# Scalsol/mega.pytorch

Hardware: NVIDIA H100
Metric: frames/sec MEGA R-101 inference (1000x600) (higher is better)
Workload: dtype f16 hi + f16 lo split operands, 3 products (near-f32) / f32 accumulate

## Files before the change

include/mega_b200.h:

```cpp
#ifndef MEGA_B200_H_
#define MEGA_B200_H_

#include <stdint.h>

#ifdef __cplusplus
extern "C" {
#endif

const char* mega_last_error(void);
int mega_abi_version(void);
int mega_device_ok(void);

typedef struct mega_conv_gemm_desc {
  const void* a;
  int a_n, a_h, a_w, a_c;
  long long a_stride_w, a_stride_h, a_stride_n;
  const void* b;
  int b_n, b_k;
  long long b_stride_n, b_stride_tap;
  int taps_r, taps_s, dil, pad;
  int k_per_tap;
  void* out;
  long long out_ld;
  int n_img, out_h, out_w, cout;
  const float* scale;
  const float* bias;
  const void* residual;
  long long res_ld;
  int relu;
  int tile_h, tile_w, block_n;
  int batch;
  int a_c_off, a_n_off;
  int b_k_off, b_n_off;
  int out_c_off, out_n_off;
  int res_c_off, res_n_off;
  int bias_z_off;
  int precision;
  int max_ctas;
  int stream_k;
  void* workspace;
  long long workspace_bytes;
  int out_f16;
  int pdl;
  int stride_h, stride_w;
  int pad_w_set, pad_w;
  long long out_stride_h, out_stride_n;
  long long res_stride_h, res_stride_n;
  int b_lo_tap_off;
  int res_split;
  float acc_scale;
  int group_width;
} mega_conv_gemm_desc;

int mega_split16_pack(const float* src, void* dst, long long n_values, void* stream);
int mega_split16_unpack(const void* src, float* dst, long long n_values, void* stream);
int mega_conv_gemm(const mega_conv_gemm_desc* desc, void* stream);
int mega_conv_gemm_tf32(const mega_conv_gemm_desc* desc, void* stream);
long long mega_conv_gemm_workspace_bytes(void);

long long mega_conv_chain_plan_bytes(int n_layers);
int mega_conv_chain_encode(const mega_conv_gemm_desc* descs, int n_layers, void* plan_host, long long plan_bytes,
                           int* grid_out);
int mega_conv_chain_launch(const void* plan_device, int n_layers, int grid, void* sync_words, void* stream, int pdl);
int mega_conv_chain_encode2(const mega_conv_gemm_desc* descs, int n_layers, void* plan_host, long long plan_bytes,
                            int* grid_out, int depth);
int mega_conv_chain_launch2(const void* plan_device, int n_layers, int grid, void* sync_words, void* stream, int pdl,
                            int depth);
int mega_conv_chain_set_trace(void* trace_dev, int cta);
int mega_conv_chain_set_trace2(void* trace_dev, int cta, int level);
int mega_set_split3_seg_len(int k_blocks);
int mega_set_tf32_rounding(int enable);

long long mega_nms_workspace_bytes(int n);
int mega_nms(const float* boxes , const float* scores , int n, float thresh, void* workspace,
             long long workspace_bytes, long long* keep_out , int* count_out, void* stream);

int mega_nms_host(const void* boxes , const void* scores , int n, float thresh, int is_double,
                  long long* keep_out , int* count_out);
int mega_roi_align_forward_nchw_host(const void* input, int batch, int channels, int height, int width, const void* rois,
                                     int num_rois, float spatial_scale, int pooled_h, int pooled_w, int sampling_ratio,
                                     int is_double, void* output);

long long mega_rpn_select_workspace_bytes(int n_img, int h, int w, int num_anchors, int pre_nms);
int mega_rpn_select(const float* head, long long head_img_stride, int ld, int n_img, int h, int w, int num_anchors,
                    int stride, const float* base_anchors, float im_w, float im_h, int pre_nms, int post_nms,
                    float nms_thresh, float min_size, void* workspace, long long workspace_bytes, float* out_boxes,
                    float* out_scores, int* out_anchor, int* out_count, void* stream);

int mega_roi_align_forward_nchw(const float* input, int batch, int channels, int height, int width,
                                const float* rois, int num_rois, float spatial_scale, int pooled_h, int pooled_w,
                                int sampling_ratio, float* output, void* stream);
int mega_roi_align_forward_nhwc(const float* input, int channels, int height, int width, long long in_img_stride,
                                const float* rois, int roi_ld, int roi_box_off, const int* roi_batch, int num_rois,
                                float spatial_scale, int pooled_h, int pooled_w, int sampling_ratio, float* output,
                                long long out_roi_stride, void* stream);

int mega_roi_align_forward_nhwc_f16(const void* input, int channels, int height, int width, long long in_img_stride,
                                    const float* rois, int roi_ld, int roi_box_off, const int* roi_batch,
                                    int num_rois, float spatial_scale, int pooled_h, int pooled_w, int sampling_ratio,
                                    void* output, long long out_roi_stride, void* stream);
int mega_roi_align_forward_nhwc_split16(const void* input, int channels, int height, int width, long long in_img_stride,
                                        const float* rois, int roi_ld, int roi_box_off, const int* roi_batch,
                                        int num_rois, float spatial_scale, int pooled_h, int pooled_w, int sampling_ratio,
                                        void* output, long long out_roi_stride, void* stream);

int mega_stem_im2col(const float* input, int n_img, int height, int width, int kpad, float* out, void* stream);
int mega_maxpool3x3s2_nhwc(const float* input, int n_img, int height, int width, int channels, float* out,
                           void* stream);
int mega_stem_im2col_f16(const float* input, int n_img, int height, int width, int kpad, void* out, void* stream);
int mega_maxpool3x3s2_nhwc_f16(const void* input, int n_img, int height, int width, int channels, void* out,
                               void* stream);
int mega_stem_prep(const float* input, int n_img, int height, int width, int wp, void* out, int f16, void* stream);
int mega_gather_rows(const float* src, long long src_ld, const int* idx, int n_rows, int row_len, float* dst,
                     long long dst_ld, void* stream);
int mega_copy_rows(const float* src, long long src_ld, const int* src_idx, float* dst, long long dst_ld,
                   const int* dst_idx, int n_rows, int row_len, void* stream);
typedef struct mega_copy_job {
  const void* src;
  long long src_ld;
  const int* src_idx;
  void* dst;
  long long dst_ld;
  const int* dst_idx;
  int n_rows;
  int row_len;
} mega_copy_job;
int mega_copy_rows_batch(const mega_copy_job* jobs_host, int n_jobs, void* stream);
int mega_transpose_2d(const float* input, int n_img, int rows, int cols, float* out, void* stream);

int mega_relation_softmax(float* logits, int n_rows, int ldm, const float* boxes_q, const float* boxes_k,
                          const float* wg, const float* bg, const float* dim_mat, const int* m_valid_ptr, int m_host,
                          const int* n_valid_ptr, int n_valid_off, float scale, void* stream);

int mega_relation_softmax_f16(float* logits, void* probs_f16, int n_rows, int ldm, const float* boxes_q,
                              const float* boxes_k, const float* wg, const float* bg, const float* dim_mat,
                              const int* m_valid_ptr, int m_host, const int* n_valid_ptr, int n_valid_off, float scale,
                              void* stream);

int mega_relation_softmax_pe(float* logits, void* probs_f16, int n_rows, int ldm, const float* boxes_q,
                             const float* boxes_k, const float* wg_host, const float* bg_host,
                             const float* dim_mat_host, const int* m_valid_ptr, int m_host, const int* n_valid_ptr,
                             int n_valid_off, float scale, void* stream);
int mega_relation_softmax_split16(float* logits, void* probs, int n_rows, int ldm, const float* boxes_q,
                                  const float* boxes_k, const float* wg, const float* bg, const float* dim_mat,
                                  const int* m_valid_ptr, int m_host, const int* n_valid_ptr, int n_valid_off, float scale,
                                  void* stream);
int mega_relation_softmax_pe_split16(float* logits, void* probs, int n_rows, int ldm, const float* boxes_q,
                                     const float* boxes_k, const float* wg_host, const float* bg_host,
                                     const float* dim_mat_host, const int* m_valid_ptr, int m_host, const int* n_valid_ptr,
                                     int n_valid_off, float scale, void* stream);

long long mega_box_postprocess_workspace_bytes(int r_max, int num_classes);
int mega_box_postprocess(const float* logits, int ld_logits, const float* deltas, int ld_deltas,
                         const float* proposals, const int* count_ptr, int r_max, int num_classes, float im_w,
                         float im_h, float score_thresh, float nms_thresh, int max_det, float wx, float wy, float ww,
                         float wh, void* workspace, long long workspace_bytes, float* out_boxes, float* out_scores,
                         long long* out_labels, int out_cap, int* out_count, void* stream);

int mega_fgfa_pool_image(const float* image, int height, int width, void* out, int f16, void* stream);
int mega_fgfa_build_pairs(const void* ring, long long slot_stride, const int* slots, int n_frames, int key_pos, int hq,
                          int wq, void* pairs, int f16, void* stream);
int mega_avgpool2_nhwc(const void* input, int n_img, int height, int width, int channels, long long in_ld, void* out,
                       long long out_ld, int f16, void* stream);
int mega_fgfa_aggregate(const void* ring, long long slot_stride, int ld, int feat_channels, int embed_channels,
                        const int* slots, int n_frames, int key_pos, const float* flow, int flow_ld, int height, int width,
                        void* out, long long out_ld, float* weights_out, int f16, void* stream);

int mega_dff_warp_scale(const void* key_feats, int ld, int channels, const float* flow, int flow_ld, const void* scale,
                        long long scale_ld, int height, int width, void* out, long long out_ld, int f16, void* stream);

int mega_sigmoid_focalloss_forward(const float* logits, const int* targets, int num_samples, int num_classes,
                                   float gamma, float alpha, float* losses, void* stream);
int mega_sigmoid_focalloss_backward(const float* logits, const int* targets, const float* d_losses, int num_samples,
                                    int num_classes, float gamma, float alpha, float* d_logits, void* stream);

int mega_deform_im2col(const float* input, const float* offset, const float* mask, int batch, int channels, int height,
                       int width, int kh, int kw, int pad_h, int pad_w, int stride_h, int stride_w, int dil_h, int dil_w,
                       int deformable_group, int kpad, float* cols, void* stream);

int mega_deform_psroi_pooling_forward(const float* input, const float* rois, const float* trans, int num_rois,
                                      int channels, int height, int width, int no_trans, float spatial_scale,
                                      int output_dim, int group_size, int pooled_size, int part_size,
                                      int sample_per_part, float trans_std, int num_classes, float* out,
                                      float* top_count, void* stream);


int mega_roi_align_backward_nchw(const float* grad, const float* rois, int num_rois, float spatial_scale, int pooled_h,
                                 int pooled_w, int batch, int channels, int height, int width, int sampling_ratio,
                                 float* grad_input, void* stream);

int mega_roi_pool_forward(const float* input, const float* rois, int num_rois, float spatial_scale, int channels,
                          int height, int width, int pooled_h, int pooled_w, float* output, int* argmax, void* stream);
int mega_roi_pool_backward(const float* grad, const int* argmax, const float* rois, int num_rois, int channels,
                           int height, int width, int pooled_h, int pooled_w, float* grad_input, void* stream);

int mega_deform_im2col_kq(const float* input, const float* offset, const float* mask, int batch, int channels,
                          int height, int width, int kh, int kw, int pad_h, int pad_w, int stride_h, int stride_w,
                          int dil_h, int dil_w, int deformable_group, int ldp, float* cols, void* stream);
int mega_deform_col2im_fused(const float* gcols, const float* input, const float* offset, const float* mask, int batch,
                             int channels, int height, int width, int kh, int kw, int pad_h, int pad_w, int stride_h,
                             int stride_w, int dil_h, int dil_w, int deformable_group, int ldp, float* grad_input,
                             float* grad_offset, float* grad_mask, void* stream);
int mega_channel_sum_nchw(const float* x, int batch, int channels, int plane, float* out, void* stream);

int mega_deform_psroi_pooling_backward(const float* out_grad, const float* input, const float* rois, const float* trans,
                                       const float* top_count, int num_rois, int channels, int height, int width,
                                       int no_trans, float spatial_scale, int output_dim, int group_size,
                                       int pooled_size, int part_size, int sample_per_part, float trans_std,
                                       int num_classes, float* input_grad, float* trans_grad, void* stream);

int mega_image_transform_u8(const unsigned char* src, int src_h, int src_w, long long src_row_stride,
                            long long src_pix_stride, long long src_ch_stride, const int* bounds_h, const int* kk_h, int ksize_h, const int* bounds_v, const int* kk_v, int ksize_v, int out_h,
                            int out_w, const float* mean_host, const float* std_host, int to_bgr255, float* out,
                            void* stream);
int mega_image_transform_u8_ex(const unsigned char* src, int src_h, int src_w, long long src_row_stride,
                               long long src_pix_stride, long long src_ch_stride, const int* bounds_h, const int* kk_h,
                               int ksize_h, const int* bounds_v, const int* kk_v, int ksize_v, int out_h, int out_w,
                               const float* mean_host, const float* std_host, int to_bgr255, int hflip, float* out,
                               void* stream);

int mega_vid_match_host(const float* pred_boxes, int n_pred, const float* gt_boxes, const unsigned char* gt_ignore,
                        int n_gt, float iou_thresh, double empty_weight, signed char* match_out,
                        double* pred_ignore_out);

long long mega_seq_nms_workspace_bytes(int num_frames, int max_det, int num_classes);
int mega_seq_nms(const float* boxes, const float* scores, const int* labels, const int* counts, int num_frames,
                 int max_det, const int* video_offsets, int num_videos, int num_classes, float link_iou, float nms_iou,
                 int rescore, void* workspace, long long workspace_bytes, float* out_scores, unsigned char* keep,
                 void* stream);

long long mega_bbox_aug_workspace_bytes(int num_passes, int r_max, int num_classes);
int mega_bbox_aug_collect(const float* logits, int ld_logits, const float* deltas, int ld_deltas, const float* proposals,
                          const int* count_ptr, int r_max, int num_classes, int pass, int num_passes, int im_w,
                          int im_h, int hflip, double ratio_w, double ratio_h, float score_thresh, float wx, float wy,
                          float ww, float wh, void* workspace, long long workspace_bytes, void* stream);
int mega_bbox_aug_merge(int num_passes, int r_max, int num_classes, float nms_thresh, int max_det, void* workspace,
                        long long workspace_bytes, float* out_boxes, float* out_scores, long long* out_labels,
                        int out_cap, int* out_count, void* stream);

#ifdef __cplusplus
}
#endif
#endif
```

mega.pytorch_b200/csrc/common.cuh:

```cuda
#pragma once
#include <cuda.h>
#include <cuda_runtime.h>
#include <stdint.h>
#include <stdio.h>

#define MEGA_OK 0
#define MEGA_ERR_ARG 1
#define MEGA_ERR_CUDA 2
#define MEGA_ERR_UNSUPPORTED 3

#define MEGA_CUDA_CHECK(expr)                                                      \
  do {                                                                             \
    cudaError_t _e = (expr);                                                       \
    if (_e != cudaSuccess) {                                                       \
      mega_set_error("%s:%d: %s -> %s", __FILE__, __LINE__, #expr,                 \
                     cudaGetErrorString(_e));                                      \
      return MEGA_ERR_CUDA;                                                        \
    }                                                                              \
  } while (0)

#define MEGA_ARG_CHECK(cond, ...)                                                  \
  do {                                                                             \
    if (!(cond)) {                                                                 \
      mega_set_error(__VA_ARGS__);                                                 \
      return MEGA_ERR_ARG;                                                         \
    }                                                                              \
  } while (0)

void mega_set_error(const char* fmt, ...);

static inline int mega_ceil_div(int a, int b) { return (a + b - 1) / b; }

#ifdef __CUDACC__
namespace mega {

__device__ __forceinline__ uint32_t smem_u32(const void* p) {
  return static_cast<uint32_t>(__cvta_generic_to_shared(p));
}

__device__ __forceinline__ uint32_t lane_id() { return threadIdx.x & 31; }

__device__ __forceinline__ bool elect_one() {
  uint32_t pred = 0;
  asm volatile(
      "{\n"
      ".reg .b32 rx;\n"
      ".reg .pred px;\n"
      "elect.sync rx|px, 0xffffffff;\n"
      "selp.b32 %0, 1, 0, px;\n"
      "}\n"
      : "=r"(pred));
  return pred != 0;
}

__device__ __forceinline__ void mbar_init(uint64_t* bar, uint32_t count) {
  asm volatile("mbarrier.init.shared::cta.b64 [%0], %1;" ::"r"(smem_u32(bar)), "r"(count));
}
__device__ __forceinline__ void fence_barrier_init() {
  asm volatile("fence.mbarrier_init.release.cluster;" ::: "memory");
}
__device__ __forceinline__ void mbar_arrive_expect_tx(uint64_t* bar, uint32_t bytes) {
  asm volatile("mbarrier.arrive.expect_tx.shared::cta.b64 _, [%0], %1;" ::"r"(smem_u32(bar)),
               "r"(bytes)
               : "memory");
}
__device__ __forceinline__ void mbar_arrive(uint64_t* bar) {
  asm volatile("mbarrier.arrive.shared::cta.b64 _, [%0];" ::"r"(smem_u32(bar)) : "memory");
}
__device__ __forceinline__ bool mbar_try_wait(uint64_t* bar, uint32_t parity) {
  uint32_t ok;
  asm volatile(
      "{\n"
      ".reg .pred p;\n"
      "mbarrier.try_wait.parity.shared::cta.b64 p, [%1], %2;\n"
      "selp.u32 %0, 1, 0, p;\n"
      "}\n"
      : "=r"(ok)
      : "r"(smem_u32(bar)), "r"(parity)
      : "memory");
  return ok != 0;
}
__device__ __forceinline__ uint64_t globaltimer_ns() {
  uint64_t t;
  asm volatile("mov.u64 %0, %%globaltimer;" : "=l"(t));
  return t;
}
__device__ __forceinline__ void mbar_wait(uint64_t* bar, uint32_t parity) {
  if (mbar_try_wait(bar, parity)) return;
#ifndef MEGA_NO_WATCHDOG
  uint64_t t0 = globaltimer_ns();
  uint32_t spins = 0;
#endif
  while (!mbar_try_wait(bar, parity)) {
#ifndef MEGA_NO_WATCHDOG
    if ((++spins & 0x3ff) == 0 && globaltimer_ns() - t0 > 2000000000ull) __trap();
#endif
  }
}

__device__ __forceinline__ void prefetch_tmap(const CUtensorMap* tm) {
  asm volatile("prefetch.tensormap [%0];" ::"l"(tm) : "memory");
}
__device__ __forceinline__ void tma_load_2d(void* dst, const CUtensorMap* tm, uint64_t* bar, int c0,
                                            int c1) {
  asm volatile(
      "cp.async.bulk.tensor.2d.shared::cluster.global.tile.mbarrier::complete_tx::bytes"
      " [%0], [%1, {%3, %4}], [%2];" ::"r"(smem_u32(dst)),
      "l"(tm), "r"(smem_u32(bar)), "r"(c0), "r"(c1)
      : "memory");
}
__device__ __forceinline__ void tma_load_3d(void* dst, const CUtensorMap* tm, uint64_t* bar, int c0,
                                            int c1, int c2) {
  asm volatile(
      "cp.async.bulk.tensor.3d.shared::cluster.global.tile.mbarrier::complete_tx::bytes"
      " [%0], [%1, {%3, %4, %5}], [%2];" ::"r"(smem_u32(dst)),
      "l"(tm), "r"(smem_u32(bar)), "r"(c0), "r"(c1), "r"(c2)
      : "memory");
}
__device__ __forceinline__ void tma_load_4d(void* dst, const CUtensorMap* tm, uint64_t* bar, int c0,
                                            int c1, int c2, int c3) {
  asm volatile(
      "cp.async.bulk.tensor.4d.shared::cluster.global.tile.mbarrier::complete_tx::bytes"
      " [%0], [%1, {%3, %4, %5, %6}], [%2];" ::"r"(smem_u32(dst)),
      "l"(tm), "r"(smem_u32(bar)), "r"(c0), "r"(c1), "r"(c2), "r"(c3)
      : "memory");
}

__device__ __forceinline__ void tma_store_4d(const CUtensorMap* tm, const void* src, int c0, int c1, int c2, int c3) {
  asm volatile(
      "cp.async.bulk.tensor.4d.global.shared::cta.bulk_group [%0, {%2, %3, %4, %5}], [%1];" ::"l"(tm),
      "r"(smem_u32(src)), "r"(c0), "r"(c1), "r"(c2), "r"(c3)
      : "memory");
}
__device__ __forceinline__ void tma_store_commit() { asm volatile("cp.async.bulk.commit_group;" ::: "memory"); }
template <int N>
__device__ __forceinline__ void tma_store_wait_read() {
  asm volatile("cp.async.bulk.wait_group.read %0;" ::"n"(N) : "memory");
}
template <int N>
__device__ __forceinline__ void tma_store_wait() {
  asm volatile("cp.async.bulk.wait_group %0;" ::"n"(N) : "memory");
}
__device__ __forceinline__ void fence_async_smem() { asm volatile("fence.proxy.async.shared::cta;" ::: "memory"); }

__device__ __forceinline__ void wgmma_fence() { asm volatile("wgmma.fence.sync.aligned;" ::: "memory"); }
__device__ __forceinline__ void wgmma_commit() { asm volatile("wgmma.commit_group.sync.aligned;" ::: "memory"); }
template <int N>
__device__ __forceinline__ void wgmma_wait() {
  asm volatile("wgmma.wait_group.sync.aligned %0;" ::"n"(N) : "memory");
}
template <int N>
__device__ __forceinline__ void wgmma_wait_regs(float (&d)[N]) {
#pragma unroll
  for (int i = 0; i < N; ++i) asm volatile("" : "+f"(d[i])::"memory");
}

template <int N>
__device__ __forceinline__ void setmaxnreg_dec() { asm volatile("setmaxnreg.dec.sync.aligned.u32 %0;" ::"n"(N)); }
template <int N>
__device__ __forceinline__ void setmaxnreg_inc() { asm volatile("setmaxnreg.inc.sync.aligned.u32 %0;" ::"n"(N)); }
__device__ __forceinline__ int ctaid_x_here() {
  int r;
  asm volatile("mov.u32 %0, %%ctaid.x;" : "=r"(r));
  return r;
}

__device__ __forceinline__ uint64_t wgmma_desc_sw128(uint32_t saddr) {
  uint64_t d = 0;
  d |= static_cast<uint64_t>((saddr & 0x3FFFFu) >> 4);
  d |= static_cast<uint64_t>(1) << 16;
  d |= static_cast<uint64_t>(1024 >> 4) << 32;
  d |= static_cast<uint64_t>(1) << 62;
  return d;
}

__device__ __forceinline__ void griddep_wait() { asm volatile("griddepcontrol.wait;" ::: "memory"); }
__device__ __forceinline__ void griddep_launch_dependents() { asm volatile("griddepcontrol.launch_dependents;" ::: "memory"); }

__device__ __forceinline__ uint32_t f2_to_h2(float lo, float hi) {
  uint32_t r;
  asm("cvt.rn.f16x2.f32 %0, %1, %2;" : "=r"(r) : "f"(hi), "f"(lo));
  return r;
}
__device__ __forceinline__ uint32_t f2_to_h2_sat(float lo, float hi) {
  uint32_t r;
  asm("cvt.rn.satfinite.f16x2.f32 %0, %1, %2;" : "=r"(r) : "f"(hi), "f"(lo));
  return r;
}
__device__ __forceinline__ float2 h2_to_f2(uint32_t h) {
  float2 f;
  asm("{\n.reg .b16 l, h;\nmov.b32 {l, h}, %2;\ncvt.f32.f16 %0, l;\ncvt.f32.f16 %1, h;\n}" : "=f"(f.x), "=f"(f.y) : "r"(h));
  return f;
}

__device__ __forceinline__ float4 ldg_f4(const float* p) {
  return __ldg(reinterpret_cast<const float4*>(p));
}

}
#endif
```

mega.pytorch_b200/csrc/conv_gemm.cu:

```cuda
#include "conv_gemm_kernel.cuh"

namespace mega {

template MEGA_LAUNCH_MODE(kModeTf32);
template MEGA_LAUNCH_MODE(kModeSplit3);

typedef CUresult (*EncodeTiledFn)(CUtensorMap*, CUtensorMapDataType, cuuint32_t, void*, const cuuint64_t*,
                                  const cuuint64_t*, const cuuint32_t*, const cuuint32_t*,
                                  CUtensorMapInterleave, CUtensorMapSwizzle, CUtensorMapL2promotion,
                                  CUtensorMapFloatOOBfill);

static EncodeTiledFn get_encode_fn() {
  static EncodeTiledFn fn = nullptr;
  if (fn) return fn;
  void* p = nullptr;
  cudaDriverEntryPointQueryResult qres;
  if (cudaGetDriverEntryPoint("cuTensorMapEncodeTiled", &p, cudaEnableDefault, &qres) != cudaSuccess ||
      qres != cudaDriverEntryPointSuccess || p == nullptr) {
    return nullptr;
  }
  fn = reinterpret_cast<EncodeTiledFn>(p);
  return fn;
}

static int g_tf32_round = 1;

static int g_num_sms = 0;
static int g_seg_len = 4;
constexpr int kCounterSlots = 65536;
constexpr int kMinUnits = 4;

}

using namespace mega;

extern "C" long long mega_conv_gemm_workspace_bytes(void) {
  return static_cast<long long>(kCounterSlots) * sizeof(int) +
         static_cast<long long>(kMaxCtas) * 2 * kBM * 256 * sizeof(float);
}

extern "C" int mega_set_split3_seg_len(int k_blocks) {
  int old = g_seg_len;
  if (k_blocks >= 1 && k_blocks <= 64) g_seg_len = k_blocks;
  return old;
}

extern "C" int mega_set_tf32_rounding(int enable) {
  int old = g_tf32_round;
  g_tf32_round = enable ? 1 : 0;
  return old;
}

namespace mega {

int encode_conv_gemm_problem(const mega_conv_gemm_desc* d, CUtensorMap* tmA_p, CUtensorMap* tmB_p, CUtensorMap* tmOut_p,
                             CUtensorMap* tmRes_p, ConvGemmParams* p_out, int* ctas_out) {
  MEGA_ARG_CHECK(d != nullptr, "conv_gemm: null descriptor");
  MEGA_ARG_CHECK(d->precision >= 0 && d->precision <= 3,
                 "conv_gemm: precision must be 0 (tf32), 1 (3xtf32), 2 (fp16 operands) or 3 (3xfp16, split-fp16 operands)");
  const bool strict = d->precision == kModeSplit3;
  const bool f16 = d->precision == kModeF16;
  const bool pk = d->precision == kModeF16x3;
  const bool out16 = d->out_f16 != 0 && !pk;
  const int esz = f16 ? 2 : 4;
  const int osz = out16 ? 2 : 4;
  const int ealign = 16 / esz, oalign = 16 / osz;
  const int bk = mode_bk(d->precision);
  MEGA_ARG_CHECK(d->tile_h > 0 && d->tile_w > 0 && d->tile_h * d->tile_w == kBM,
                 "conv_gemm: tile_h*tile_w must be 128 (got %dx%d)", d->tile_h, d->tile_w);
  MEGA_ARG_CHECK(d->tile_w <= 256 && d->tile_h <= 256, "conv_gemm: tile too large for a TMA box");
  const int stride_h = d->stride_h > 0 ? d->stride_h : 1, stride_w = d->stride_w > 0 ? d->stride_w : 1;
  MEGA_ARG_CHECK((d->tile_w - 1) * stride_w + 1 <= 256 && (d->tile_h - 1) * stride_h + 1 <= 256,
                 "conv_gemm: strided tile %dx%d (stride %dx%d) exceeds the 256-element TMA box", d->tile_h, d->tile_w,
                 stride_h, stride_w);
  MEGA_ARG_CHECK(d->block_n == 32 || d->block_n == 64 || d->block_n == 96 || d->block_n == 128 ||
                     d->block_n == 160 || d->block_n == 192 || d->block_n == 256,
                 "conv_gemm: block_n must be one of 32/64/96/128/160/192/256");
  MEGA_ARG_CHECK(!out16 || (f16 && d->block_n % 64 == 0),
                 "conv_gemm: fp16 output needs fp16 operands and block_n %% 64 == 0 (got precision %d, block_n %d)",
                 d->precision, d->block_n);
  MEGA_ARG_CHECK((reinterpret_cast<uintptr_t>(d->a) & 15) == 0 && (reinterpret_cast<uintptr_t>(d->b) & 15) == 0,
                 "conv_gemm: operand base pointers must be 16-byte aligned");
  MEGA_ARG_CHECK((d->a_stride_w % ealign) == 0 && (d->a_stride_h % ealign) == 0 && (d->a_stride_n % ealign) == 0,
                 "conv_gemm: activation strides must be multiples of 16 bytes");
  MEGA_ARG_CHECK(d->out != nullptr && (reinterpret_cast<uintptr_t>(d->out) & 15) == 0 && (d->out_ld % oalign) == 0,
                 "conv_gemm: output must be 16-byte aligned with a row pitch multiple of 16 bytes");
  MEGA_ARG_CHECK(d->residual == nullptr ||
                     ((reinterpret_cast<uintptr_t>(d->residual) & 15) == 0 && (d->res_ld % oalign) == 0),
                 "conv_gemm: residual must be 16-byte aligned with a row pitch multiple of 16 bytes");
  MEGA_ARG_CHECK(d->out_c_off == 0 || d->cout == d->block_n,
                 "conv_gemm: channel-offset batching needs cout == block_n (got %d vs %d)", d->cout, d->block_n);
  MEGA_ARG_CHECK((d->b_stride_n % ealign) == 0 && (d->b_stride_tap % ealign) == 0,
                 "conv_gemm: weight strides must be multiples of 16 bytes");
  MEGA_ARG_CHECK(d->batch >= 1, "conv_gemm: batch must be >= 1");
  MEGA_ARG_CHECK(d->workspace != nullptr && d->workspace_bytes >= mega_conv_gemm_workspace_bytes(),
                 "conv_gemm: workspace missing or smaller than mega_conv_gemm_workspace_bytes()");
  MEGA_ARG_CHECK((reinterpret_cast<uintptr_t>(d->workspace) & 255) == 0, "conv_gemm: workspace must be 256-byte aligned");
  EncodeTiledFn enc = get_encode_fn();
  if (!enc) {
    mega_set_error("conv_gemm: cuTensorMapEncodeTiled unavailable (no CUDA driver?)");
    return MEGA_ERR_CUDA;
  }
  MEGA_ARG_CHECK(!(strict || pk) || d->block_n == 64 || d->block_n == 128, "conv_gemm: 3xtf32 / 3xfp16 support block_n 64 / 128");
  if (pk) {
    MEGA_ARG_CHECK((d->a_c & 31) == 0 && (d->b_k & 31) == 0 && (d->k_per_tap & 31) == 0 && (d->a_c_off & 31) == 0 &&
                       (d->b_k_off & 31) == 0,
                   "conv_gemm: split-fp16 operands need channel counts / offsets in multiples of 32 (a_c %d, b_k %d, k %d)",
                   d->a_c, d->b_k, d->k_per_tap);
    const int cout_r = (d->cout + 31) & ~31;
    MEGA_ARG_CHECK(d->out_f16 == 0 || ((d->out_c_off & 31) == 0 && (d->cout == cout_r || (d->batch == 1 && d->out_ld >= cout_r))),
                   "conv_gemm: split-fp16 output needs cout (%d) in multiples of 32 (or batch 1 and a row pitch >= the rounded cout)", d->cout);
    MEGA_ARG_CHECK(d->res_split == 0 || d->residual == nullptr ||
                       ((d->res_c_off & 31) == 0 && (d->cout == cout_r || (d->batch == 1 && d->res_ld >= cout_r))),
                   "conv_gemm: split-fp16 residual needs cout (%d) in multiples of 32", d->cout);
    MEGA_ARG_CHECK((d->a_stride_w & 31) == 0 && (d->b_stride_n & 31) == 0 && (reinterpret_cast<uintptr_t>(d->a) & 127) == 0 &&
                       (reinterpret_cast<uintptr_t>(d->b) & 127) == 0,
                   "conv_gemm: split-fp16 operands need 128-byte aligned rows");
    MEGA_ARG_CHECK(d->scale == nullptr,
                   "conv_gemm: precision 3 takes no per-channel scale: fold it into the weights before packing them "
                   "(mega_core.b200.ops.pack_weights_split16(w, scale))");
  } else {
    MEGA_ARG_CHECK(d->res_split == 0, "conv_gemm: res_split needs precision 3");
  }
  if (d->group_width != 0) {
    const int gw = d->group_width;
    MEGA_ARG_CHECK(gw == 8 || gw == 16 || gw == 32 || gw == 64, "conv_gemm: group_width must be 8, 16, 32 or 64 (got %d)", gw);
    MEGA_ARG_CHECK(d->block_n == 64 && d->cout == 64 && d->k_per_tap == 64 && d->b_k == 64 && d->a_c_off == 64 &&
                       d->b_n_off == 64 && d->out_c_off == 64 && d->b_k_off == 0 && (d->residual == nullptr || d->res_c_off == 64),
                   "conv_gemm: group_width needs the 64-channel batched layout (block_n = cout = k_per_tap = b_k = 64, "
                   "a_c_off = b_n_off = out_c_off = res_c_off = 64, b_k_off = 0; got block_n %d cout %d k %d b_k %d offsets "
                   "%d %d %d %d %d)", d->block_n, d->cout, d->k_per_tap, d->b_k, d->a_c_off, d->b_n_off, d->out_c_off,
                   d->res_c_off, d->b_k_off);
    MEGA_ARG_CHECK(d->b_lo_tap_off == 0, "conv_gemm: group_width does not take pre-split weights (b_lo_tap_off)");
  }
  const CUtensorMapDataType dt = f16 ? CU_TENSOR_MAP_DATA_TYPE_FLOAT16
                                     : (g_tf32_round && !strict && !pk) ? CU_TENSOR_MAP_DATA_TYPE_TFLOAT32
                                                                 : CU_TENSOR_MAP_DATA_TYPE_FLOAT32;
  const CUtensorMapDataType odt = out16 ? CU_TENSOR_MAP_DATA_TYPE_FLOAT16 : CU_TENSOR_MAP_DATA_TYPE_FLOAT32;

  CUtensorMap& tmA = *tmA_p;
  CUtensorMap& tmB = *tmB_p;
  {
    cuuint64_t gdim[4] = {static_cast<cuuint64_t>(d->a_c), static_cast<cuuint64_t>(d->a_w),
                          static_cast<cuuint64_t>(d->a_h), static_cast<cuuint64_t>(d->a_n)};
    cuuint64_t gstr[3] = {static_cast<cuuint64_t>(d->a_stride_w) * esz, static_cast<cuuint64_t>(d->a_stride_h) * esz,
                          static_cast<cuuint64_t>(d->a_stride_n) * esz};
    cuuint32_t box[4] = {static_cast<cuuint32_t>(bk), static_cast<cuuint32_t>((d->tile_w - 1) * stride_w + 1),
                         static_cast<cuuint32_t>((d->tile_h - 1) * stride_h + 1), 1};
    cuuint32_t estr[4] = {1, static_cast<cuuint32_t>(stride_w), static_cast<cuuint32_t>(stride_h), 1};
    CUresult r = enc(&tmA, dt, 4, const_cast<void*>(d->a), gdim, gstr, box, estr, CU_TENSOR_MAP_INTERLEAVE_NONE,
                     CU_TENSOR_MAP_SWIZZLE_128B, CU_TENSOR_MAP_L2_PROMOTION_L2_256B,
                     CU_TENSOR_MAP_FLOAT_OOB_FILL_NONE);
    if (r != CUDA_SUCCESS) {
      mega_set_error("conv_gemm: encode A tensor map failed (CUresult %d) dims %d %d %d %d strides %lld %lld %lld",
                     static_cast<int>(r), d->a_c, d->a_w, d->a_h, d->a_n, d->a_stride_w, d->a_stride_h,
                     d->a_stride_n);
      return MEGA_ERR_CUDA;
    }
  }
  {
    const int taps = d->taps_r * d->taps_s;
    MEGA_ARG_CHECK(d->b_lo_tap_off == 0 || (strict && d->b_lo_tap_off == taps && d->batch == 1),
                   "conv_gemm: b_lo_tap_off (%d) needs precision 1, batch 1 and must equal taps_r * taps_s (%d)",
                   d->b_lo_tap_off, taps);
    cuuint64_t gdim[3] = {static_cast<cuuint64_t>(d->b_k), static_cast<cuuint64_t>(d->b_n),
                          static_cast<cuuint64_t>(taps + d->b_lo_tap_off)};
    cuuint64_t gstr[2] = {static_cast<cuuint64_t>(d->b_stride_n) * esz,
                          static_cast<cuuint64_t>((taps > 1 || d->b_lo_tap_off) && d->b_stride_tap > 0
                                                      ? d->b_stride_tap : d->b_stride_n * d->b_n) * esz};
    cuuint32_t box[3] = {static_cast<cuuint32_t>(bk), static_cast<cuuint32_t>(pass_n(d->block_n)), 1};
    cuuint32_t estr[3] = {1, 1, 1};
    CUresult r = enc(&tmB, dt, 3, const_cast<void*>(d->b), gdim, gstr, box, estr, CU_TENSOR_MAP_INTERLEAVE_NONE,
                     CU_TENSOR_MAP_SWIZZLE_128B, CU_TENSOR_MAP_L2_PROMOTION_L2_256B,
                     CU_TENSOR_MAP_FLOAT_OOB_FILL_NONE);
    if (r != CUDA_SUCCESS) {
      mega_set_error("conv_gemm: encode B tensor map failed (CUresult %d) dims %d %d %d strides %lld %lld",
                     static_cast<int>(r), d->b_k, d->b_n, taps, d->b_stride_n, d->b_stride_tap);
      return MEGA_ERR_CUDA;
    }
  }

  CUtensorMap& tmOut = *tmOut_p;
  CUtensorMap& tmRes = *tmRes_p;
  int out_cext = 0, out_tail0 = 0;
  long long out_str_h = 0, out_str_n = 0;
  {
    const int box_w = d->tile_w < 32 ? d->tile_w : 32;
    const int box_h = 32 / box_w;
    const int cw = out16 ? 64 : 32;
    for (int which = 0; which < 2; ++which) {
      const void* base = which == 0 ? d->out : d->residual;
      CUtensorMap* tm = which == 0 ? &tmOut : &tmRes;
      if (base == nullptr) {
        *tm = tmOut;
        continue;
      }
      const long long ld = which == 0 ? d->out_ld : d->res_ld;
      const int c_off = which == 0 ? d->out_c_off : d->res_c_off;
      const int n_off = which == 0 ? d->out_n_off : d->res_n_off;
      const bool split_fmt = pk && (which == 0 ? d->out_f16 != 0 : d->res_split != 0);
      const int c_extent = (split_fmt ? ((d->cout + 31) & ~31) : d->cout) + (d->batch - 1) * c_off;
      const int c_tail0 = (c_extent * osz / 16) * 16 / osz;
      if (which == 0) {
        out_cext = c_extent;
        out_tail0 = c_tail0;
      }
      const int c_map = (which == 0 && c_tail0 > 0) ? c_tail0 : c_extent;
      cuuint64_t gdim[4] = {static_cast<cuuint64_t>(c_map), static_cast<cuuint64_t>(d->out_w),
                            static_cast<cuuint64_t>(d->out_h),
                            static_cast<cuuint64_t>(d->n_img + (d->batch - 1) * n_off)};
      const long long sh = which == 0 ? d->out_stride_h : d->res_stride_h;
      const long long sn = which == 0 ? d->out_stride_n : d->res_stride_n;
      const long long str_h = sh > 0 ? sh : ld * d->out_w;
      const long long str_n = sn > 0 ? sn : str_h * d->out_h;
      MEGA_ARG_CHECK((str_h % oalign) == 0 && (str_n % oalign) == 0, "conv_gemm: output strides must be multiples of 16 bytes");
      if (which == 0) {
        out_str_h = str_h;
        out_str_n = str_n;
      }
      cuuint64_t gstr[3] = {static_cast<cuuint64_t>(ld) * osz, static_cast<cuuint64_t>(str_h) * osz,
                            static_cast<cuuint64_t>(str_n) * osz};
      cuuint32_t box[4] = {static_cast<cuuint32_t>(cw), static_cast<cuuint32_t>(box_w), static_cast<cuuint32_t>(box_h), 1};
      cuuint32_t estr[4] = {1, 1, 1, 1};
      CUresult r = enc(tm, odt, 4, const_cast<void*>(base), gdim, gstr, box, estr,
                       CU_TENSOR_MAP_INTERLEAVE_NONE, CU_TENSOR_MAP_SWIZZLE_128B, CU_TENSOR_MAP_L2_PROMOTION_L2_256B,
                       CU_TENSOR_MAP_FLOAT_OOB_FILL_NONE);
      if (r != CUDA_SUCCESS) {
        mega_set_error("conv_gemm: encode %s tensor map failed (CUresult %d): C %d W %d H %d N %d ld %lld",
                       which == 0 ? "output" : "residual", static_cast<int>(r), static_cast<int>(gdim[0]), d->out_w,
                       d->out_h, static_cast<int>(gdim[3]), ld);
        return MEGA_ERR_CUDA;
      }
    }
  }

  ConvGemmParams& p = *p_out;
  p.tile_w = d->tile_w;
  p.tile_h = d->tile_h;
  p.tiles_w = mega_ceil_div(d->out_w, d->tile_w);
  p.tiles_h = mega_ceil_div(d->out_h, d->tile_h);
  p.out_h = d->out_h;
  p.out_w = d->out_w;
  p.n_img = d->n_img;
  p.taps_r = d->taps_r;
  p.taps_s = d->taps_s;
  p.dil = d->dil;
  p.pad = d->pad;
  p.pad_w = d->pad_w_set ? d->pad_w : d->pad;
  p.stride_h = stride_h;
  p.stride_w = stride_w;
  p.k_chunks = mega_ceil_div(d->k_per_tap, bk);
  p.cout = d->cout;
  p.scale = d->scale;
  p.bias = d->bias;
  p.has_residual = d->residual != nullptr;
  p.relu = d->relu;
  p.a_c_off = d->a_c_off;
  p.a_n_off = d->a_n_off;
  p.b_k_off = d->b_k_off;
  p.b_n_off = d->b_n_off;
  p.out_c_off = d->out_c_off;
  p.out_n_off = d->out_n_off;
  p.res_c_off = d->res_c_off;
  p.res_n_off = d->res_n_off;
  p.bias_z_off = d->bias_z_off;
  p.box_w = d->tile_w < 32 ? d->tile_w : 32;
  p.box_h = 32 / p.box_w;
  p.m_tiles = p.tiles_w * p.tiles_h * p.n_img;
  p.n_tiles = mega_ceil_div(d->cout, d->block_n);
  p.kb_per_tile = d->taps_r * d->taps_s * p.k_chunks;
  const long long tiles = static_cast<long long>(d->batch) * p.m_tiles * p.n_tiles;
  p.total_units = tiles * p.kb_per_tile;
  p.total_tiles = tiles;
  p.stream_k = d->stream_k ? 1 : 0;
  p.seg_len = g_seg_len;
  p.b_lo_tap_off = d->b_lo_tap_off;
  p.res_split = d->res_split ? 1 : 0;
  p.acc_scale = (pk && d->acc_scale != 0.f) ? d->acc_scale : 1.f;
  p.out_ptr = d->out;
  p.out_ld = d->out_ld;
  p.out_str_h = out_str_h;
  p.out_str_n = out_str_n;
  p.out_tail0 = out_tail0;
  p.out_cext = out_cext;
  MEGA_ARG_CHECK(tiles <= kCounterSlots, "conv_gemm: %lld output tiles exceed the %d counter slots", tiles, kCounterSlots);
  MEGA_ARG_CHECK(p.total_units > 0, "conv_gemm: empty problem");
  MEGA_ARG_CHECK(p.total_units * kMaxCtas < (1LL << 31), "conv_gemm: %lld work units exceed the 32-bit work-list range",
                 p.total_units);
  p.counters = static_cast<int*>(d->workspace);
  p.part_ws = reinterpret_cast<float*>(static_cast<char*>(d->workspace) + kCounterSlots * sizeof(int));
  if (g_num_sms == 0) {
    int dev = 0;
    MEGA_CUDA_CHECK(cudaGetDevice(&dev));
    MEGA_CUDA_CHECK(cudaDeviceGetAttribute(&g_num_sms, cudaDevAttrMultiProcessorCount, dev));
    if (g_num_sms > kMaxCtas) g_num_sms = kMaxCtas;
  }
  long long ctas = p.stream_k ? p.total_units / kMinUnits : tiles;
  if (ctas < 1) ctas = 1;
  if (ctas > g_num_sms) ctas = g_num_sms;
  if (d->max_ctas > 0 && ctas > d->max_ctas) ctas = d->max_ctas;
  if (p.stream_k && p.kb_per_tile >= 256 && tiles <= ctas) {
    const long long aligned = (ctas / tiles) * tiles;
    if (aligned * 100 >= ctas * 85) ctas = aligned;
  }
  *ctas_out = static_cast<int>(ctas);
  return MEGA_OK;
}

}

extern "C" int mega_conv_gemm(const mega_conv_gemm_desc* d, void* stream_v) {
  cudaStream_t stream = static_cast<cudaStream_t>(stream_v);
  CUtensorMap tmA, tmB, tmOut, tmRes;
  ConvGemmParams p;
  int ctas = 0;
  const int erc = encode_conv_gemm_problem(d, &tmA, &tmB, &tmOut, &tmRes, &p, &ctas);
  if (erc != MEGA_OK) return erc;
  const bool out16 = d->out_f16 != 0;
  dim3 grid(static_cast<unsigned>(ctas), 1, 1);
  const int pdl = d->pdl ? 1 : 0;
  const int gw = d->group_width == 64 ? 0 : d->group_width;
  switch (d->precision) {
    case kModeTf32: return launch_mode<kModeTf32>(d->block_n, out16, gw, tmA, tmB, tmOut, tmRes, p, grid, stream, pdl);
    case kModeSplit3: return launch_mode<kModeSplit3>(d->block_n, out16, gw, tmA, tmB, tmOut, tmRes, p, grid, stream, pdl);
    case kModeF16: return launch_mode<kModeF16>(d->block_n, out16, gw, tmA, tmB, tmOut, tmRes, p, grid, stream, pdl);
    default: return launch_mode<kModeF16x3>(d->block_n, out16, gw, tmA, tmB, tmOut, tmRes, p, grid, stream, pdl);
  }
}

extern "C" int mega_conv_gemm_tf32(const mega_conv_gemm_desc* d, void* stream) { return mega_conv_gemm(d, stream); }
```

mega.pytorch_b200/csrc/conv_gemm_kernel.cuh:

```cuda
#include "common.cuh"
#pragma once
#include "mega_b200.h"
#include "wgmma.cuh"

namespace mega {

constexpr int kBM = 128;
constexpr int kModeTf32 = 0;
constexpr int kModeSplit3 = 1;
constexpr int kModeF16 = 2;
constexpr int kModeF16x3 = 3;
__host__ __device__ constexpr int mode_bk(int mode) { return mode == kModeF16 ? 64 : 32; }
constexpr int kThreads = 192;
constexpr int kMaxCtas = 132;
constexpr int kRingSlots = 2;
constexpr int kRingSlotBytes = kBM * 128;
__host__ __device__ constexpr int mma_warp0(int mode) { return mode == kModeSplit3 ? 12 : 8; }
__host__ __device__ constexpr int conv_gemm_threads(int mode) { return (mma_warp0(mode) + 8) * 32; }
constexpr int kF16x3RegsProducer = 40, kF16x3RegsEpilogue = 104, kF16x3RegsMma = 184;
static_assert(128 * kF16x3RegsProducer + 128 * kF16x3RegsEpilogue + 256 * kF16x3RegsMma == 65536 &&
                  conv_gemm_threads(kModeF16x3) == 512,
              "3xFP16 register split");
__host__ __device__ constexpr int pass_n(int bn) { return bn <= 128 ? bn : (bn == 160 ? 96 : bn / 2); }
constexpr int conv_gemm_stages(int mode, int bn) {
  if (mode == kModeSplit3) return bn == 64 ? 4 : 2;
  if (mode == kModeF16x3) return bn == 64 ? 5 : 4;
  return bn == 32 ? 6 : bn == 64 ? 5 : bn <= 128 ? 4 : bn <= 192 ? 3 : 2;
}

struct ConvGemmParams {
  int tiles_w, tiles_h, tile_w, tile_h;
  int out_h, out_w, n_img;
  int taps_r, taps_s, dil, pad;
  int pad_w;
  int stride_h, stride_w;
  int k_chunks;
  int cout;
  const float* scale;
  const float* bias;
  int has_residual;
  int relu;
  int a_c_off, a_n_off, b_k_off, b_n_off;
  int out_c_off, out_n_off;
  int res_c_off, res_n_off;
  int bias_z_off;
  int box_w, box_h;
  int m_tiles, n_tiles;
  int kb_per_tile;
  long long total_units;
  long long total_tiles;
  int stream_k;
  float* part_ws;
  int* counters;
  int seg_len;
  int b_lo_tap_off;
  int res_split;
  float acc_scale;
  void* out_ptr;
  long long out_ld, out_str_h, out_str_n;
  int out_tail0, out_cext;
};

template <int BN, int STAGES, int MODE = kModeTf32>
struct SmemLayout {
  static constexpr bool SPLIT3 = MODE == kModeSplit3;
  static constexpr int kABytes = kBM * 128;
  static constexpr int kBBytes = pass_n(BN) * 128;
  static constexpr int kHalf = kABytes + kBBytes;
  static constexpr int kStageBytes = SPLIT3 ? kHalf + kBBytes : kHalf;
  static constexpr int kRingOffset = STAGES * kStageBytes;
  static constexpr int kEpiOffset = kRingOffset + kRingSlots * kRingSlotBytes;
  static constexpr int kEpiBytes = 4 * 4 * 4096;
  static constexpr int kBarOffset = kEpiOffset + kEpiBytes;
  static constexpr int kSbCols = BN <= 128 ? 128 : 256;
  static constexpr int kSbOffset = kBarOffset + 512;
  static constexpr int kTotal = kSbOffset + 8 * kSbCols + 1024;
};

struct TileCoord {
  int img, h0, w0, n0, batch;
};

__device__ __forceinline__ TileCoord decode_tile(const ConvGemmParams& p, int t, int bn) {
  TileCoord c;
  const int m_tile = t % p.m_tiles;
  const int rest = t / p.m_tiles;
  const int n_tile = rest % p.n_tiles;
  c.batch = rest / p.n_tiles;
  const int tw_i = m_tile % p.tiles_w;
  const int th_i = (m_tile / p.tiles_w) % p.tiles_h;
  c.img = m_tile / (p.tiles_w * p.tiles_h);
  c.h0 = th_i * p.tile_h;
  c.w0 = tw_i * p.tile_w;
  c.n0 = n_tile * bn;
  return c;
}

__device__ __forceinline__ int cta_first_unit(int total, int grid, int c) {
  return static_cast<int>((static_cast<unsigned>(total) * static_cast<unsigned>(c)) / static_cast<unsigned>(grid));
}

__device__ __forceinline__ int unit_owner(int total, int grid, int u) {
  int c = static_cast<int>((static_cast<unsigned>(u) * static_cast<unsigned>(grid)) / static_cast<unsigned>(total));
  if (c >= grid) c = grid - 1;
  while (c + 1 < grid && cta_first_unit(total, grid, c + 1) <= u) ++c;
  while (c > 0 && cta_first_unit(total, grid, c) > u) --c;
  return c;
}

struct WorkIter {
  int u, u_end, tile, tiles;
  int KB, grid;
  bool sk;
  __device__ __forceinline__ WorkIter(const ConvGemmParams& p, int cta, int grid_)
      : tile(cta), tiles(static_cast<int>(p.total_tiles)), KB(p.kb_per_tile), grid(grid_), sk(p.stream_k != 0) {
    u = cta_first_unit(static_cast<int>(p.total_units), grid_, cta);
    u_end = cta_first_unit(static_cast<int>(p.total_units), grid_, cta + 1);
  }
  __device__ __forceinline__ bool next(int& t, int& kb0, int& kb1) {
    if (sk) {
      if (u >= u_end) return false;
      t = u / KB;
      kb0 = u - t * KB;
      kb1 = min(KB, kb0 + (u_end - u));
      u += kb1 - kb0;
      return true;
    }
    if (tile >= tiles) return false;
    t = tile;
    kb0 = 0;
    kb1 = KB;
    tile += grid;
    return true;
  }
};

template <int THREADS>
__device__ __forceinline__ void epi_bar_sync() { asm volatile("bar.sync 1, %0;" ::"n"(THREADS) : "memory"); }

__device__ __forceinline__ float* sk_part_row(const ConvGemmParams& p, int c, int slot, int row, int bn) {
  return p.part_ws + ((static_cast<long long>(c) * 2 + slot) * kBM + row) * bn;
}

__device__ __forceinline__ float* sk_own_part_row(const ConvGemmParams& p, int cta, int tile_item, int row, int bn) {
  return sk_part_row(p, cta, tile_item == 0 ? 0 : 1, row, bn);
}

__device__ __forceinline__ void sk_publish(float* part, int col0, const uint32_t (&acc)[32]) {
  float* ws = part + col0;
#pragma unroll
  for (int j = 0; j < 32; j += 4)
    __stcg(reinterpret_cast<float4*>(ws + j), make_float4(__uint_as_float(acc[j]), __uint_as_float(acc[j + 1]),
                                                          __uint_as_float(acc[j + 2]), __uint_as_float(acc[j + 3])));
}

template <int THREADS>
__device__ __forceinline__ bool sk_elect_finisher(const ConvGemmParams& p, int U, int grid, int KB, int t, int epi_tid,
                                                  int* flag, int& c_first, int& c_last) {
  __threadfence();
  epi_bar_sync<THREADS>();
  c_first = unit_owner(U, grid, t * KB);
  c_last = unit_owner(U, grid, t * KB + KB - 1);
  if (epi_tid == 0) {
    const int parts = c_last - c_first + 1;
    const int old = atomicAdd(&p.counters[t], 1);
    const int last = (old == parts - 1);
    if (last) p.counters[t] = 0;
    *flag = last;
  }
  epi_bar_sync<THREADS>();
  const bool finisher = *flag != 0;
  if (finisher) __threadfence();
  return finisher;
}

__device__ __forceinline__ void sk_reduce(const ConvGemmParams& p, int U, int grid, int KB, int t, int c_first, int c_last,
                                          int row, int bn, int col0, float (&acc)[32]) {
#pragma unroll
  for (int j = 0; j < 32; ++j) acc[j] = 0.f;
  for (int oc = c_first; oc <= c_last; ++oc) {
    const int slot = (cta_first_unit(U, grid, oc) >= t * KB) ? 0 : 1;
    const float* ws = sk_part_row(p, oc, slot, row, bn) + col0;
#pragma unroll
    for (int j = 0; j < 32; j += 4) {
      const float4 v = __ldcg(reinterpret_cast<const float4*>(ws + j));
      acc[j] += v.x; acc[j + 1] += v.y; acc[j + 2] += v.z; acc[j + 3] += v.w;
    }
  }
}

struct StoreBox {
  int w, h, res_n;
};
__device__ __forceinline__ StoreBox store_box(const ConvGemmParams& p, const TileCoord& tc, int q) {
  const int r0 = q * 32;
  const int bh0 = r0 / p.tile_w, bw0 = r0 - bh0 * p.tile_w;
  return {tc.w0 + bw0, tc.h0 + bh0, tc.img + tc.batch * p.res_n_off};
}

template <bool HALF>
__device__ __forceinline__ void store_tail(const ConvGemmParams& p, const uint8_t* rowp, int gc0, int cw, const StoreBox& box,
                                          int out_n, int lane) {
  const int h = box.h + lane / p.box_w, w = box.w + lane % p.box_w;
  if (h >= p.out_h || w >= p.out_w) return;
  const int j0 = max(p.out_tail0 - gc0, 0), j1 = min(p.out_cext - gc0, cw);
  const uint32_t sw = static_cast<uint32_t>(lane & 7);
  const long long pix = static_cast<long long>(out_n) * p.out_str_n + static_cast<long long>(h) * p.out_str_h +
                        static_cast<long long>(w) * p.out_ld + gc0;
  for (int j = j0; j < j1; ++j) {
    if (HALF)
      static_cast<uint16_t*>(p.out_ptr)[pix + j] =
          *reinterpret_cast<const uint16_t*>(rowp + ((static_cast<uint32_t>(j >> 3) ^ sw) << 4) + (j & 7) * 2);
    else
      static_cast<float*>(p.out_ptr)[pix + j] =
          *reinterpret_cast<const float*>(rowp + ((static_cast<uint32_t>(j >> 2) ^ sw) << 4) + (j & 3) * 4);
  }
}

__device__ __forceinline__ void stage_scale_bias(float* sb, int bias_off, const ConvGemmParams& p, const TileCoord& tc, int i) {
  const int n = tc.n0 + i;
  const int zoff = tc.batch * p.bias_z_off;
  sb[i] = (p.scale && n < p.cout) ? __ldg(p.scale + zoff + n) : 1.f;
  sb[bias_off + i] = (p.bias && n < p.cout) ? __ldg(p.bias + zoff + n) : 0.f;
}

struct PipeState {
  int stage;
  uint32_t phase;
};

template <int STAGES, class F>
__device__ __forceinline__ void produce_pass(const CUtensorMap* tmA, const CUtensorMap* tmB, uint64_t* full_bar,
                                             uint64_t* empty_bar, PipeState& ps, uint8_t* stage0, int stage_bytes, int b_off,
                                             int b_lo_off, int bk, uint32_t tx_bytes, const ConvGemmParams& p,
                                             const TileCoord& tc, int n0, int kb0, int kb1, int lane, F&& on_stage) {
  const int k_chunks = p.k_chunks, taps_s = p.taps_s;
  int tap = kb0 / k_chunks;
  int kc = kb0 - tap * k_chunks;
  int r = tap / taps_s;
  int sx = tap - r * taps_s;
  const int a_c0 = tc.batch * p.a_c_off, a_n = tc.img + tc.batch * p.a_n_off;
  const int b_k0 = tc.batch * p.b_k_off, b_n = n0 + tc.batch * p.b_n_off;
  for (int kb = kb0; kb < kb1; ++kb) {
    mbar_wait(&empty_bar[ps.stage], ps.phase ^ 1);
    on_stage(kb);
    uint8_t* dst = stage0 + ps.stage * stage_bytes;
    if (lane == 0) {
      mbar_arrive_expect_tx(&full_bar[ps.stage], tx_bytes);
      tma_load_4d(dst, tmA, &full_bar[ps.stage], kc * bk + a_c0, tc.w0 * p.stride_w + sx * p.dil - p.pad_w,
                  tc.h0 * p.stride_h + r * p.dil - p.pad, a_n);
    } else {
      tma_load_3d(dst + b_off, tmB, &full_bar[ps.stage], kc * bk + b_k0, b_n, tap);
      if (b_lo_off != 0) tma_load_3d(dst + b_lo_off, tmB, &full_bar[ps.stage], kc * bk + b_k0, b_n, tap + p.b_lo_tap_off);
    }
    if (++kc == k_chunks) {
      kc = 0;
      ++tap;
      if (++sx == taps_s) {
        sx = 0;
        ++r;
      }
    }
    if (++ps.stage == STAGES) {
      ps.stage = 0;
      ps.phase ^= 1;
    }
  }
}

__device__ __forceinline__ void ring_take(const uint8_t* ring, uint64_t* full, uint64_t* empty, uint32_t slot, uint32_t use,
                                          int row, uint32_t (&r)[32]) {
  mbar_wait(&full[slot], use & 1u);
  const uint8_t* rowp = ring + slot * kRingSlotBytes + row * 128;
#pragma unroll
  for (int j = 0; j < 8; ++j) {
    const uint4 v = *reinterpret_cast<const uint4*>(rowp + ((j ^ (row & 7)) << 4));
    r[4 * j] = v.x; r[4 * j + 1] = v.y; r[4 * j + 2] = v.z; r[4 * j + 3] = v.w;
  }
  __syncwarp();
  if ((threadIdx.x & 31) == 0) mbar_arrive(&empty[slot]);
}
__device__ __forceinline__ void ring_take(const uint8_t* ring, uint64_t* full, uint64_t* empty, uint32_t seq, int row,
                                          uint32_t (&r)[32]) {
  ring_take(ring, full, empty, seq % kRingSlots, seq / kRingSlots, row, r);
}
__device__ __forceinline__ void ring_skip(const uint8_t* ring, uint64_t* full, uint64_t* empty, uint32_t slot, uint32_t use,
                                          int row) {
  uint32_t r[32];
  ring_take(ring, full, empty, slot, use, row, r);
}
__device__ __forceinline__ void ring_skip(const uint8_t* ring, uint64_t* full, uint64_t* empty, uint32_t seq, int row) {
  ring_skip(ring, full, empty, seq % kRingSlots, seq / kRingSlots, row);
}

template <int NR>
__device__ __forceinline__ void ring_put(uint8_t* ring, uint64_t* full, uint64_t* empty, uint32_t slot, uint32_t use, int wg,
                                         int wtid, const float (&d)[NR], const int c) {
  if (use > 0) mbar_wait(&empty[slot], (use - 1) & 1u);
  const int r0 = wg * 64 + (wtid >> 5) * 16 + ((wtid & 31) >> 2);
  const int t = wtid & 3;
  uint8_t* base = ring + slot * kRingSlotBytes;
#pragma unroll
  for (int i = 0; i < 4; ++i) {
    const int j = 2 * i + (t >> 1);
    const int off = (t & 1) * 8;
    *reinterpret_cast<float2*>(base + r0 * 128 + ((j ^ (r0 & 7)) << 4) + off) =
        make_float2(d[4 * (4 * c + i)], d[4 * (4 * c + i) + 1]);
    const int r1 = r0 + 8;
    *reinterpret_cast<float2*>(base + r1 * 128 + ((j ^ (r1 & 7)) << 4) + off) =
        make_float2(d[4 * (4 * c + i) + 2], d[4 * (4 * c + i) + 3]);
  }
  mbar_arrive(&full[slot]);
}

template <int BN, int MODE>
__device__ __forceinline__ void mma_kblock(float (&d)[BN / 2], uint32_t a_addr, uint32_t b_addr, uint32_t b_lo_addr,
                                           const int wtid, const bool first) {
  const uint64_t adesc = wgmma_desc_sw128(a_addr);
  const uint64_t bdesc = wgmma_desc_sw128(b_addr);
  if constexpr (MODE == kModeSplit3) {
    const int g = (wtid >> 5) * 16 + ((wtid & 31) >> 2), t = wtid & 3;
    const uint64_t blo = wgmma_desc_sw128(b_lo_addr);
    uint32_t ahi[4][4], alo[4][4];
#pragma unroll
    for (int k = 0; k < 4; ++k) {
#pragma unroll
      for (int e = 0; e < 4; ++e) {
        const int r = g + (e & 1) * 8, col = 8 * k + t + (e >> 1) * 4;
        float x;
        asm volatile("ld.shared.f32 %0, [%1];" : "=f"(x) : "r"(a_addr + r * 128 + ((((col >> 2) ^ (r & 7)) << 4) | ((col & 3) << 2))));
        const uint32_t h = __float_as_uint(x) & 0xffffe000u;
        ahi[k][e] = h;
        alo[k][e] = __float_as_uint(x - __uint_as_float(h));
      }
    }
    wgmma_fence();
#pragma unroll
    for (int k = 0; k < 4; ++k) {
      Wgmma<BN>::tf32_rs(d, ahi[k], bdesc + 2 * k, (first && k == 0) ? 0 : 1);
      Wgmma<BN>::tf32_rs(d, ahi[k], blo + 2 * k, 1);
      Wgmma<BN>::tf32_rs(d, alo[k], bdesc + 2 * k, 1);
    }
  } else if constexpr (MODE == kModeF16x3) {
    wgmma_fence();
#pragma unroll
    for (int k = 0; k < 2; ++k) {
      Wgmma<BN>::f16_ss(d, adesc + 2 * k, bdesc + 2 * k, (first && k == 0) ? 0 : 1);
      Wgmma<BN>::f16_ss(d, adesc + 2 * k, bdesc + 4 + 2 * k, 1);
      Wgmma<BN>::f16_ss(d, adesc + 4 + 2 * k, bdesc + 2 * k, 1);
    }
  } else {
    wgmma_fence();
#pragma unroll
    for (int k = 0; k < 4; ++k) {
      if (MODE == kModeF16) Wgmma<BN>::f16_ss(d, adesc + 2 * k, bdesc + 2 * k, (first && k == 0) ? 0 : 1);
      else Wgmma<BN>::tf32_ss(d, adesc + 2 * k, bdesc + 2 * k, (first && k == 0) ? 0 : 1);
    }
  }
  wgmma_commit();
}

template <int V>
struct IntC {
  static constexpr int value = V;
};
template <int K, int KN, class F>
__device__ __forceinline__ void static_for(F&& f) {
  if constexpr (K < KN) {
    f(IntC<K>());
    static_for<K + 1, KN>(f);
  }
}

template <int MODE, int GW, int KC>
__device__ __forceinline__ void mma_kblock_grouped(float (&d)[32], uint32_t a_addr, uint32_t b_addr, uint32_t b_lo_addr,
                                                   const int wtid) {
  constexpr int KS = (MODE == kModeF16 || MODE == kModeF16x3) ? 16 : 8;
  constexpr int N = GW > KS ? GW : KS;
  constexpr int NK = MODE == kModeF16x3 ? 2 : 4;
  const uint64_t adesc = wgmma_desc_sw128(a_addr);
  const uint64_t bdesc = wgmma_desc_sw128(b_addr);
  if constexpr (MODE == kModeSplit3) {
    const int g = (wtid >> 5) * 16 + ((wtid & 31) >> 2), t = wtid & 3;
    const uint64_t blo = wgmma_desc_sw128(b_lo_addr);
    uint32_t ahi[4][4], alo[4][4];
#pragma unroll
    for (int k = 0; k < 4; ++k) {
#pragma unroll
      for (int e = 0; e < 4; ++e) {
        const int r = g + (e & 1) * 8, col = 8 * k + t + (e >> 1) * 4;
        float x;
        asm volatile("ld.shared.f32 %0, [%1];" : "=f"(x) : "r"(a_addr + r * 128 + ((((col >> 2) ^ (r & 7)) << 4) | ((col & 3) << 2))));
        const uint32_t h = __float_as_uint(x) & 0xffffe000u;
        ahi[k][e] = h;
        alo[k][e] = __float_as_uint(x - __uint_as_float(h));
      }
    }
    wgmma_fence();
    static_for<0, NK>([&](auto kc) {
      constexpr int k = decltype(kc)::value;
      constexpr int col0 = (32 * KC + KS * k) / N * N;
      float(&dd)[N / 2] = *reinterpret_cast<float(*)[N / 2]>(&d[col0 / 2]);
      Wgmma<N>::tf32_rs(dd, ahi[k], bdesc + 2 * k + 8 * col0, 1);
      Wgmma<N>::tf32_rs(dd, ahi[k], blo + 2 * k + 8 * col0, 1);
      Wgmma<N>::tf32_rs(dd, alo[k], bdesc + 2 * k + 8 * col0, 1);
    });
  } else {
    wgmma_fence();
    static_for<0, NK>([&](auto kc) {
      constexpr int k = decltype(kc)::value;
      constexpr int col0 = (32 * KC + KS * k) / N * N;
      float(&dd)[N / 2] = *reinterpret_cast<float(*)[N / 2]>(&d[col0 / 2]);
      if constexpr (MODE == kModeF16x3) {
        Wgmma<N>::f16_ss(dd, adesc + 2 * k, bdesc + 2 * k + 8 * col0, 1);
        Wgmma<N>::f16_ss(dd, adesc + 2 * k, bdesc + 4 + 2 * k + 8 * col0, 1);
        Wgmma<N>::f16_ss(dd, adesc + 4 + 2 * k, bdesc + 2 * k + 8 * col0, 1);
      } else if constexpr (MODE == kModeF16) {
        Wgmma<N>::f16_ss(dd, adesc + 2 * k, bdesc + 2 * k + 8 * col0, 1);
      } else {
        Wgmma<N>::tf32_ss(dd, adesc + 2 * k, bdesc + 2 * k + 8 * col0, 1);
      }
    });
  }
  wgmma_commit();
}

template <int MODE, int GW>
__device__ __forceinline__ void mma_kblock_grouped(float (&d)[32], uint32_t a_addr, uint32_t b_addr, uint32_t b_lo_addr,
                                                   const int wtid, const int kb) {
  if (mode_bk(MODE) == 64 || (kb & 1) == 0) mma_kblock_grouped<MODE, GW, 0>(d, a_addr, b_addr, b_lo_addr, wtid);
  else mma_kblock_grouped<MODE, GW, 1>(d, a_addr, b_addr, b_lo_addr, wtid);
}

struct MmaState {
  int stage;
  uint32_t phase;
  uint32_t uses[kRingSlots];
};

template <int PN, int STAGES, int MODE, class L, int GW = 0>
__device__ __forceinline__ void mma_pass(uint8_t* smem, uint64_t* full_bar, uint64_t* empty_bar, uint64_t* split_bar,
                                         uint8_t* ring, uint64_t* ring_full, uint64_t* ring_empty, MmaState& ms, int kb0,
                                         int kb1, int seg_len, int wg, int wtid, int hpc) {
  static_assert(GW == 0 || PN == 64, "grouped k-blocks need a 64-column pass");
  constexpr bool SPLIT3 = MODE == kModeSplit3;
  constexpr bool SEG = SPLIT3 || MODE == kModeF16x3;
  const int lane = wtid & 31;
  float d[PN / 2];
  float master[SEG ? PN / 2 : 1];
  if constexpr (MODE == kModeF16x3) {
#pragma unroll
    for (int i = 0; i < PN / 2; ++i) master[i] = -0.f;
  }
  bool has_master = false;
  for (int s0 = kb0, s1 = 0; s0 < kb1; s0 = s1) {
    s1 = (kb1 - s0 > seg_len) ? s0 + seg_len : kb1;
    int pending = -1;
    if constexpr (GW > 0) {
#pragma unroll
      for (int i = 0; i < PN / 2; ++i) d[i] = 0.f;
    }
    for (int kb = s0; kb < s1; ++kb) {
      mbar_wait(SPLIT3 ? &split_bar[ms.stage] : &full_bar[ms.stage], ms.phase);
      const uint32_t a_addr = smem_u32(smem + ms.stage * L::kStageBytes);
      if constexpr (GW > 0)
        mma_kblock_grouped<MODE, GW>(d, a_addr + wg * 64 * 128, a_addr + L::kABytes, a_addr + L::kABytes + L::kBBytes, wtid,
                                     kb);
      else
        mma_kblock<PN, MODE>(d, a_addr + wg * 64 * 128, a_addr + L::kABytes, a_addr + L::kABytes + L::kBBytes, wtid, kb == s0);
      if (SPLIT3) wgmma_wait<0>(); else wgmma_wait<1>();
      if (pending >= 0) {
        __syncwarp();
        if (lane == 0) mbar_arrive(&empty_bar[pending]);
      }
      pending = ms.stage;
      if (++ms.stage == STAGES) {
        ms.stage = 0;
        ms.phase ^= 1;
      }
    }
    wgmma_wait<0>();
    wgmma_wait_regs(d);
    if (pending >= 0) {
      __syncwarp();
      if (lane == 0) mbar_arrive(&empty_bar[pending]);
    }
    if constexpr (MODE == kModeF16x3) {
#pragma unroll
      for (int i = 0; i < PN / 2; ++i) master[i] = __fadd_rn(d[i], master[i]);
    } else if constexpr (SEG) {
#pragma unroll
      for (int i = 0; i < PN / 2; ++i) master[i] = has_master ? __fadd_rn(d[i], master[i]) : d[i];
      has_master = true;
    }
  }
#pragma unroll
  for (int c = 0; c < PN / 32; ++c) {
    uint32_t slot;
    if (hpc == 0) slot = (ms.uses[0] == ms.uses[1]) ? 0u : 1u;
    else slot = static_cast<uint32_t>((c / hpc) & 1);
    const uint32_t use = ms.uses[slot]++;
    if constexpr (SEG) ring_put(ring, ring_full, ring_empty, slot, use, wg, wtid, master, c);
    else ring_put(ring, ring_full, ring_empty, slot, use, wg, wtid, d, c);
  }
}

template <int BN, int STAGES, int MODE, bool OUT16, int GW = 0>
__global__ void __launch_bounds__(conv_gemm_threads(MODE), 1)
conv_gemm_kernel(const __grid_constant__ CUtensorMap tmA, const __grid_constant__ CUtensorMap tmB,
                      const __grid_constant__ CUtensorMap tmOut, const __grid_constant__ CUtensorMap tmRes,
                      const ConvGemmParams p) {
  constexpr bool SPLIT3 = MODE == kModeSplit3;
  constexpr bool PK = MODE == kModeF16x3;
  constexpr bool SEG = SPLIT3 || PK;
  constexpr bool OUTH = OUT16 && !PK;
  constexpr int kBK = mode_bk(MODE);
  constexpr int CW = OUTH ? 64 : 32;
  constexpr int kMmaWarp0 = mma_warp0(MODE);
  static_assert(!OUTH || BN % 64 == 0, "fp16 output needs block_n % 64 == 0");
  static_assert(SmemLayout<BN, STAGES, MODE>::kTotal <= 227 * 1024, "pipeline + staging exceed the 227 KB of a CTA");
  using L = SmemLayout<BN, STAGES, MODE>;
  const int kSegLen = SEG ? p.seg_len : 0x7fffffff;
  extern __shared__ uint8_t smem_raw[];
  uint8_t* smem = reinterpret_cast<uint8_t*>((reinterpret_cast<uintptr_t>(smem_raw) + 1023) &
                                             ~static_cast<uintptr_t>(1023));
  uint64_t* full_bar = reinterpret_cast<uint64_t*>(smem + L::kBarOffset);
  uint64_t* empty_bar = full_bar + STAGES;
  uint64_t* split_bar = empty_bar + STAGES;
  uint64_t* ring_full = split_bar + STAGES;
  uint64_t* ring_empty = ring_full + kRingSlots;
  uint64_t* res_bar = ring_empty + kRingSlots;
  int* epi_flag = reinterpret_cast<int*>(res_bar + 16);
  uint8_t* ring = smem + L::kRingOffset;

  const int warp = threadIdx.x >> 5;
  const int lane = threadIdx.x & 31;
  const int grid = gridDim.x;
  const int cta = blockIdx.x;
  const int U = static_cast<int>(p.total_units);
  const int KB = p.kb_per_tile;

  if (warp == 0 && lane == 0) {
    prefetch_tmap(&tmA);
    prefetch_tmap(&tmB);
    prefetch_tmap(&tmOut);
    if (p.has_residual) prefetch_tmap(&tmRes);
  }
  if (warp == 1 && lane == 0) {
    for (int s = 0; s < STAGES; ++s) {
      mbar_init(&full_bar[s], 1);
      mbar_init(&empty_bar[s], 8);
      mbar_init(&split_bar[s], 4);
    }
    for (int b = 0; b < kRingSlots; ++b) {
      mbar_init(&ring_full[b], 256);
      mbar_init(&ring_empty[b], 4);
    }
    for (int b = 0; b < 16; ++b) mbar_init(&res_bar[b], 1);
    fence_barrier_init();
  }
  __syncthreads();
  griddep_wait();
  griddep_launch_dependents();
  if (warp == 0) {
    if (PK) setmaxnreg_dec<kF16x3RegsProducer>();
    if (lane < 2) {
      PipeState ps = {0, 0};
      WorkIter it(p, PK ? ctaid_x_here() : cta, grid);
      int t;
      int kb0, kb1;
      const bool b_lo = SPLIT3 && p.b_lo_tap_off > 0;
      while (it.next(t, kb0, kb1)) {
        const TileCoord tc = decode_tile(p, t, BN);
        for (int pass = 0; pass < (BN > pass_n(BN) ? 2 : 1); ++pass)
          produce_pass<STAGES>(&tmA, &tmB, full_bar, empty_bar, ps, smem, L::kStageBytes, L::kABytes,
                               b_lo ? L::kABytes + L::kBBytes : 0, kBK, L::kHalf + (b_lo ? L::kBBytes : 0), p, tc,
                               tc.n0 + pass * pass_n(BN), kb0, kb1, lane, [](int) {});
      }
    }
  } else if (warp >= kMmaWarp0) {
    if (PK) setmaxnreg_inc<kF16x3RegsMma>();
    const int wg = (warp - kMmaWarp0) >> 2;
    const int wtid = threadIdx.x - (kMmaWarp0 + 4 * wg) * 32;
    constexpr int P0 = pass_n(BN), P1 = BN - P0;
    MmaState ms = {0, 0, {0, 0}};
    WorkIter it(p, PK ? ctaid_x_here() : cta, grid);
    int t;
    int kb0, kb1;
    while (it.next(t, kb0, kb1)) {
      mma_pass<P0, STAGES, MODE, L, GW>(smem, full_bar, empty_bar, split_bar, ring, ring_full, ring_empty, ms, kb0, kb1,
                                        kSegLen, wg, wtid, 0);
      if constexpr (P1 > 0)
        mma_pass<P1, STAGES, MODE, L>(smem, full_bar, empty_bar, split_bar, ring, ring_full, ring_empty, ms, kb0, kb1,
                                      kSegLen, wg, wtid, 0);
    }
  } else if (warp >= 6 && warp < 10 && !PK) {
    if (SPLIT3) {
      const int stid = threadIdx.x - kThreads;
      int stage = 0;
      uint32_t phase = 0;
      WorkIter it(p, cta, grid);
      int t;
      int kb0, kb1;
      const bool need_lo = p.b_lo_tap_off == 0;
      while (it.next(t, kb0, kb1)) {
        for (int kb = kb0; kb < kb1; ++kb) {
          mbar_wait(&full_bar[stage], phase);
          uint8_t* bb = smem + stage * L::kStageBytes + L::kABytes;
          constexpr int kVecs = L::kBBytes / 16;
#pragma unroll 4
          for (int v = stid; v < kVecs; v += 128) {
            float4 x = *reinterpret_cast<const float4*>(bb + v * 16);
            float4 h;
            h.x = __uint_as_float(__float_as_uint(x.x) & 0xffffe000u);
            h.y = __uint_as_float(__float_as_uint(x.y) & 0xffffe000u);
            h.z = __uint_as_float(__float_as_uint(x.z) & 0xffffe000u);
            h.w = __uint_as_float(__float_as_uint(x.w) & 0xffffe000u);
            *reinterpret_cast<float4*>(bb + v * 16) = h;
            if (need_lo)
              *reinterpret_cast<float4*>(bb + L::kBBytes + v * 16) = make_float4(x.x - h.x, x.y - h.y, x.z - h.z, x.w - h.w);
          }
          fence_async_smem();
          __syncwarp();
          if (lane == 0) mbar_arrive(&split_bar[stage]);
          if (++stage == STAGES) {
            stage = 0;
            phase ^= 1;
          }
        }
      }
    }
  } else if (PK && warp >= 4 && warp < 8) {
    setmaxnreg_dec<kF16x3RegsEpilogue>();
    constexpr int kCPW = BN / 32;
    const int q = warp & 3;
    const int row = q * 32 + lane;
    const int epi_tid = (warp - 4) * 32 + lane;
    uint8_t* stage_buf = smem + L::kEpiOffset + (warp - 4) * (kCPW * 4096);
    uint64_t* rbar = res_bar + (warp - 4) * 4;
    float* bias_s = reinterpret_cast<float*>(smem + L::kSbOffset);
    uint32_t rphase = 0;
    const int cta_e = ctaid_x_here();
    WorkIter it(p, cta_e, grid);
    int t;
    int kb0, kb1;
    uint32_t seq0 = 0;
    const uint32_t sw = static_cast<uint32_t>(lane & 7);
    const bool res_split = p.res_split != 0;
    const float slope = p.relu == 2 ? 0.1f : 0.f;
    for (int tile_item = 0; it.next(t, kb0, kb1); ++tile_item, seq0 += BN / 32) {
      const TileCoord tc = decode_tile(p, t, BN);
      const bool complete = (kb0 == 0 && kb1 == KB);
      const StoreBox box = store_box(p, tc, q);
      const int nchunks = min(BN / 32, (p.cout - tc.n0 + 31) / 32);
      const int bsel = tile_item & 1;
      epi_bar_sync<128>();
      if (tile_item == 0) {
        if (epi_tid < BN) {
          const int n = tc.n0 + epi_tid;
          bias_s[epi_tid] = (p.bias && n < p.cout) ? __ldg(p.bias + tc.batch * p.bias_z_off + n) : 0.f;
        }
        epi_bar_sync<128>();
      }
      float next_bias = 0.f;
      bool has_next = false;
      {
        WorkIter peek = it;
        int t2, k0, k1;
        has_next = peek.next(t2, k0, k1);
        if (has_next && epi_tid < BN) {
          const TileCoord tc2 = decode_tile(p, t2, BN);
          const int n = tc2.n0 + epi_tid;
          next_bias = (p.bias && n < p.cout) ? __ldg(p.bias + tc2.batch * p.bias_z_off + n) : 0.f;
        }
      }
      if (lane == 0) tma_store_wait_read<0>();
      __syncwarp();
      auto issue_residual = [&]() {
        if (p.has_residual && lane == 0) {
#pragma unroll
          for (int j = 0; j < kCPW; ++j) {
            if (j < nchunks) {
              mbar_arrive_expect_tx(&rbar[j], 4096);
              tma_load_4d(stage_buf + j * 4096, &tmRes, &rbar[j], tc.n0 + j * 32 + tc.batch * p.res_c_off, box.w, box.h,
                          box.res_n);
            }
          }
        }
      };
      if (complete) issue_residual();
      auto load_chunk = [&](const int j, float (&acc)[32]) {
        uint32_t raw[32];
        ring_take(ring, ring_full, ring_empty, seq0 + j, row, raw);
#pragma unroll
        for (int i = 0; i < 32; ++i) acc[i] = __uint_as_float(raw[i]);
      };
      bool finalize = complete;
      int c_first = cta_e, c_last = cta_e;
      if (!complete) {
        float* part = sk_own_part_row(p, cta_e, tile_item, row, BN);
#pragma unroll
        for (int j = 0; j < kCPW; ++j) {
          uint32_t raw[32];
          ring_take(ring, ring_full, ring_empty, seq0 + j, row, raw);
          sk_publish(part, j * 32, raw);
        }
        finalize = sk_elect_finisher<128>(p, U, grid, KB, t, epi_tid, epi_flag, c_first, c_last);
        if (finalize) issue_residual();
      }
      if (finalize) {
        const int out_n = tc.img + tc.batch * p.out_n_off;
#pragma unroll
        for (int j = 0; j < kCPW; ++j) {
          if (j < nchunks) {
            float acc[32];
            if (complete) load_chunk(j, acc);
            else sk_reduce(p, U, grid, KB, t, c_first, c_last, row, BN, j * 32, acc);
            uint8_t* rowp = stage_buf + j * 4096 + lane * 128;
            const float4* biv = reinterpret_cast<const float4*>(bias_s + bsel * BN + j * 32);
#pragma unroll
            for (int i = 0; i < 32; i += 4) {
              const float4 bi = biv[i >> 2];
              acc[i] = fmaf(acc[i], p.acc_scale, bi.x); acc[i + 1] = fmaf(acc[i + 1], p.acc_scale, bi.y);
              acc[i + 2] = fmaf(acc[i + 2], p.acc_scale, bi.z); acc[i + 3] = fmaf(acc[i + 3], p.acc_scale, bi.w);
            }
            if (p.has_residual) {
              mbar_wait(&rbar[j], (rphase >> j) & 1u);
              rphase ^= (1u << j);
              if (res_split) {
#pragma unroll
                for (int c = 0; c < 4; ++c) {
                  const uint4 rh = *reinterpret_cast<const uint4*>(rowp + ((static_cast<uint32_t>(c) ^ sw) << 4));
                  const uint4 rl = *reinterpret_cast<const uint4*>(rowp + ((static_cast<uint32_t>(4 + c) ^ sw) << 4));
                  const uint32_t hs[4] = {rh.x, rh.y, rh.z, rh.w}, ls[4] = {rl.x, rl.y, rl.z, rl.w};
#pragma unroll
                  for (int e = 0; e < 4; ++e) {
                    const float2 a2 = h2_to_f2(hs[e]), b2 = h2_to_f2(ls[e]);
                    acc[8 * c + 2 * e] += a2.x + b2.x;
                    acc[8 * c + 2 * e + 1] += a2.y + b2.y;
                  }
                }
              } else {
#pragma unroll
                for (int c = 0; c < 8; ++c) {
                  const float4 rr = *reinterpret_cast<const float4*>(rowp + ((static_cast<uint32_t>(c) ^ sw) << 4));
                  acc[4 * c] += rr.x; acc[4 * c + 1] += rr.y; acc[4 * c + 2] += rr.z; acc[4 * c + 3] += rr.w;
                }
              }
            }
            if (p.relu) {
#pragma unroll
              for (int i = 0; i < 32; ++i) acc[i] = fmaxf(acc[i], slope * acc[i]);
            }
            if (OUT16) {
#pragma unroll
              for (int c = 0; c < 4; ++c) {
                uint32_t hh[4], ll[4];
#pragma unroll
                for (int e = 0; e < 4; ++e) {
                  hh[e] = f2_to_h2_sat(acc[8 * c + 2 * e], acc[8 * c + 2 * e + 1]);
                  const float2 back = h2_to_f2(hh[e]);
                  ll[e] = f2_to_h2_sat(acc[8 * c + 2 * e] - back.x, acc[8 * c + 2 * e + 1] - back.y);
                }
                *reinterpret_cast<uint4*>(rowp + ((static_cast<uint32_t>(c) ^ sw) << 4)) = make_uint4(hh[0], hh[1], hh[2], hh[3]);
                *reinterpret_cast<uint4*>(rowp + ((static_cast<uint32_t>(4 + c) ^ sw) << 4)) = make_uint4(ll[0], ll[1], ll[2], ll[3]);
              }
            } else {
#pragma unroll
              for (int c = 0; c < 8; ++c)
                *reinterpret_cast<float4*>(rowp + ((static_cast<uint32_t>(c) ^ sw) << 4)) =
                    make_float4(acc[4 * c], acc[4 * c + 1], acc[4 * c + 2], acc[4 * c + 3]);
            }
            fence_async_smem();
            __syncwarp();
            const int gc0 = tc.n0 + j * 32 + tc.batch * p.out_c_off;
            if (!OUT16 && gc0 + 32 > p.out_tail0) store_tail<false>(p, rowp, gc0, 32, box, out_n, lane);
            if (lane == 0 && gc0 < p.out_tail0) {
              tma_store_4d(&tmOut, stage_buf + j * 4096, gc0, box.w, box.h, out_n);
              tma_store_commit();
            }
          } else if (complete) {
            ring_skip(ring, ring_full, ring_empty, seq0 + j, row);
          }
        }
      }
      if (has_next && epi_tid < BN) bias_s[(bsel ^ 1) * BN + epi_tid] = next_bias;
    }
    if (lane == 0) tma_store_wait<0>();
  } else if (PK) {
    setmaxnreg_dec<kF16x3RegsProducer>();
  } else if (warp >= 2 && warp < 6) {
    const int q = warp & 3;
    const int row = q * 32 + lane;
    const int epi_tid = (warp - 2) * 32 + lane;
    uint8_t* epi_out = smem + L::kEpiOffset + (warp - 2) * 16384;
    uint8_t* epi_res = epi_out + 8192;
    uint64_t* rbar = res_bar + (warp - 2) * 2;
    float* sb_s = reinterpret_cast<float*>(smem + L::kSbOffset);
    uint32_t rphase = 0;
    WorkIter it(p, cta, grid);
    int t;
    int kb0, kb1;
    uint32_t seq0 = 0;
    for (int tile_item = 0; it.next(t, kb0, kb1); ++tile_item, seq0 += BN / 32) {
      const TileCoord tc = decode_tile(p, t, BN);
      const bool complete = (kb0 == 0 && kb1 == KB);
      const StoreBox box = store_box(p, tc, q);
      const int nchunks = min(BN / CW, (p.cout - tc.n0 + CW - 1) / CW);
      epi_bar_sync<128>();
      for (int i = epi_tid; i < BN; i += 128) stage_scale_bias(sb_s, L::kSbCols, p, tc, i);
      if (complete && p.has_residual && lane == 0 && nchunks > 0) {
        mbar_arrive_expect_tx(&rbar[0], 4096);
        tma_load_4d(epi_res, &tmRes, &rbar[0], tc.n0 + tc.batch * p.res_c_off, box.w, box.h, box.res_n);
      }
      epi_bar_sync<128>();
      bool finalize = complete;
      int c_first = cta, c_last = cta;
      if (!complete) {
        float* part = sk_own_part_row(p, cta, tile_item, row, BN);
#pragma unroll 1
        for (int c = 0; c < BN / 32; ++c) {
          uint32_t raw[32];
          ring_take(ring, ring_full, ring_empty, seq0 + c, row, raw);
          sk_publish(part, c * 32, raw);
        }
        finalize = sk_elect_finisher<128>(p, U, grid, KB, t, epi_tid, epi_flag, c_first, c_last);
      }
      if (finalize) {
        const int out_n = tc.img + tc.batch * p.out_n_off;
        const bool has_sb = (p.scale != nullptr) || (p.bias != nullptr);
        const uint32_t sw = static_cast<uint32_t>(lane & 7);
        if (!complete && p.has_residual && lane == 0 && nchunks > 0) {
          mbar_arrive_expect_tx(&rbar[0], 4096);
          tma_load_4d(epi_res, &tmRes, &rbar[0], tc.n0 + tc.batch * p.res_c_off, box.w, box.h, box.res_n);
        }
        auto finish_chunk = [&](const int c) {
          const int nb = tc.n0 + c * CW;
          const uint8_t* rsrc = nullptr;
          if (p.has_residual) {
            const int rb = c & 1;
            if (c + 1 < nchunks && lane == 0) {
              mbar_arrive_expect_tx(&rbar[rb ^ 1], 4096);
              tma_load_4d(epi_res + (rb ^ 1) * 4096, &tmRes, &rbar[rb ^ 1], nb + CW + tc.batch * p.res_c_off, box.w, box.h,
                          box.res_n);
            }
            mbar_wait(&rbar[rb], (rphase >> rb) & 1u);
            rphase ^= (1u << rb);
            rsrc = epi_res + rb * 4096 + lane * 128;
          }
          if (lane == 0) tma_store_wait_read<1>();
          __syncwarp();
          uint8_t* dst = epi_out + (c & 1) * 4096 + lane * 128;
        #pragma unroll
          for (int h = 0; h < CW / 32; ++h) {
            const int col0 = c * CW + h * 32;
            float acc[32];
            if (complete) {
              uint32_t raw[32];
              ring_take(ring, ring_full, ring_empty, seq0 + col0 / 32, row, raw);
        #pragma unroll
              for (int j = 0; j < 32; ++j) acc[j] = __uint_as_float(raw[j]);
            } else {
              sk_reduce(p, U, grid, KB, t, c_first, c_last, row, BN, col0, acc);
            }
            if (has_sb) {
              const float4* scv = reinterpret_cast<const float4*>(sb_s + col0);
              const float4* biv = reinterpret_cast<const float4*>(sb_s + L::kSbCols + col0);
        #pragma unroll
              for (int j = 0; j < 32; j += 4) {
                const float4 sc = scv[j >> 2], bi = biv[j >> 2];
                acc[j] = fmaf(acc[j], sc.x, bi.x); acc[j + 1] = fmaf(acc[j + 1], sc.y, bi.y);
                acc[j + 2] = fmaf(acc[j + 2], sc.z, bi.z); acc[j + 3] = fmaf(acc[j + 3], sc.w, bi.w);
              }
            }
            const float slope = p.relu == 2 ? 0.1f : 0.f;
            if (OUTH) {
        #pragma unroll
              for (int j = 0; j < 32; j += 8) {
                const uint32_t chunk = (static_cast<uint32_t>((h * 32 + j) >> 3) ^ sw) << 4;
                float v[8];
        #pragma unroll
                for (int e = 0; e < 8; ++e) v[e] = acc[j + e];
                if (rsrc) {
                  const uint4 rr = *reinterpret_cast<const uint4*>(rsrc + chunk);
                  const float2 r0v = h2_to_f2(rr.x), r1v = h2_to_f2(rr.y), r2v = h2_to_f2(rr.z), r3v = h2_to_f2(rr.w);
                  v[0] += r0v.x; v[1] += r0v.y; v[2] += r1v.x; v[3] += r1v.y;
                  v[4] += r2v.x; v[5] += r2v.y; v[6] += r3v.x; v[7] += r3v.y;
                }
                if (p.relu) {
        #pragma unroll
                  for (int e = 0; e < 8; ++e) v[e] = fmaxf(v[e], slope * v[e]);
                }
                uint4 o;
                o.x = f2_to_h2(v[0], v[1]); o.y = f2_to_h2(v[2], v[3]);
                o.z = f2_to_h2(v[4], v[5]); o.w = f2_to_h2(v[6], v[7]);
                *reinterpret_cast<uint4*>(dst + chunk) = o;
              }
            } else {
        #pragma unroll
              for (int j = 0; j < 32; j += 4) {
                float4 v = make_float4(acc[j], acc[j + 1], acc[j + 2], acc[j + 3]);
                const uint32_t chunk = (static_cast<uint32_t>(j >> 2) ^ sw) << 4;
                if (rsrc) {
                  const float4 rr = *reinterpret_cast<const float4*>(rsrc + chunk);
                  v.x += rr.x; v.y += rr.y; v.z += rr.z; v.w += rr.w;
                }
                if (p.relu) {
                  v.x = fmaxf(v.x, slope * v.x); v.y = fmaxf(v.y, slope * v.y);
                  v.z = fmaxf(v.z, slope * v.z); v.w = fmaxf(v.w, slope * v.w);
                }
                *reinterpret_cast<float4*>(dst + chunk) = v;
              }
            }
          }
          fence_async_smem();
          __syncwarp();
          const int gc0 = nb + tc.batch * p.out_c_off;
          if (gc0 + CW > p.out_tail0) store_tail<OUTH>(p, dst, gc0, CW, box, out_n, lane);
          if (lane == 0 && gc0 < p.out_tail0) {
            tma_store_4d(&tmOut, epi_out + (c & 1) * 4096, gc0, box.w, box.h, out_n);
            tma_store_commit();
          }
        };
#pragma unroll 1
        for (int c = 0; c < nchunks; ++c) finish_chunk(c);
      }
      if (complete) {
#pragma unroll 1
        for (int c = nchunks * (CW / 32); c < BN / 32; ++c) ring_skip(ring, ring_full, ring_empty, seq0 + c, row);
      }
    }
    if (lane == 0) tma_store_wait<0>();
  }
}

template <int BN, int STAGES, int MODE, bool OUT16, int GW = 0>
static int launch_cfg(const CUtensorMap& tmA, const CUtensorMap& tmB, const CUtensorMap& tmOut,
                      const CUtensorMap& tmRes, const ConvGemmParams& p, dim3 grid, cudaStream_t stream, int pdl) {
  using L = SmemLayout<BN, STAGES, MODE>;
  static bool configured = false;
  if (!configured) {
    MEGA_CUDA_CHECK(cudaFuncSetAttribute(conv_gemm_kernel<BN, STAGES, MODE, OUT16, GW>,
                                         cudaFuncAttributeMaxDynamicSharedMemorySize, L::kTotal));
    configured = true;
  }
  cudaLaunchConfig_t cfg = {};
  cfg.gridDim = grid;
  cfg.blockDim = dim3(conv_gemm_threads(MODE), 1, 1);
  cfg.dynamicSmemBytes = L::kTotal;
  cfg.stream = stream;
  cudaLaunchAttribute attr[1];
  attr[0].id = cudaLaunchAttributeProgrammaticStreamSerialization;
  attr[0].val.programmaticStreamSerializationAllowed = 1;
  cfg.attrs = attr;
  cfg.numAttrs = pdl ? 1 : 0;
  MEGA_CUDA_CHECK(cudaLaunchKernelEx(&cfg, conv_gemm_kernel<BN, STAGES, MODE, OUT16, GW>, tmA, tmB, tmOut, tmRes, p));
  return MEGA_OK;
}

template <int MODE>
int launch_mode(int block_n, bool out16, int gw, const CUtensorMap& tmA, const CUtensorMap& tmB, const CUtensorMap& tmOut,
                const CUtensorMap& tmRes, const ConvGemmParams& p, dim3 grid, cudaStream_t stream, int pdl) {
  auto launch = [&](auto bn, auto gw_c) -> int {
    constexpr int BN = decltype(bn)::value, GW = decltype(gw_c)::value, ST = conv_gemm_stages(MODE, BN);
    if constexpr (MODE == kModeF16x3 || (MODE == kModeF16 && BN % 64 == 0)) {
      if (out16) return launch_cfg<BN, ST, MODE, true, GW>(tmA, tmB, tmOut, tmRes, p, grid, stream, pdl);
    } else if (out16) {
      mega_set_error("conv_gemm: fp16 output needs fp16 operands and block_n %% 64 == 0 (got precision %d, block_n %d)",
                     MODE, BN);
      return MEGA_ERR_ARG;
    }
    return launch_cfg<BN, ST, MODE, false, GW>(tmA, tmB, tmOut, tmRes, p, grid, stream, pdl);
  };
  switch (gw) {
    case 8: return launch(IntC<64>(), IntC<8>());
    case 16: return launch(IntC<64>(), IntC<16>());
    case 32: return launch(IntC<64>(), IntC<32>());
  }
  switch (block_n) {
    case 64: return launch(IntC<64>(), IntC<0>());
    case 128: return launch(IntC<128>(), IntC<0>());
  }
  if constexpr (MODE == kModeTf32 || MODE == kModeF16) {
    switch (block_n) {
      case 32: return launch(IntC<32>(), IntC<0>());
      case 96: return launch(IntC<96>(), IntC<0>());
      case 160: return launch(IntC<160>(), IntC<0>());
      case 192: return launch(IntC<192>(), IntC<0>());
      case 256: return launch(IntC<256>(), IntC<0>());
    }
  }
  mega_set_error("conv_gemm: unsupported block_n %d for precision %d", block_n, MODE);
  return MEGA_ERR_ARG;
}

#define MEGA_LAUNCH_MODE(M)                                                                                                \
  int launch_mode<M>(int, bool, int, const CUtensorMap&, const CUtensorMap&, const CUtensorMap&, const CUtensorMap&,     \
                     const ConvGemmParams&, dim3, cudaStream_t, int)
extern template MEGA_LAUNCH_MODE(kModeTf32);
extern template MEGA_LAUNCH_MODE(kModeSplit3);
extern template MEGA_LAUNCH_MODE(kModeF16);
extern template MEGA_LAUNCH_MODE(kModeF16x3);

}
```

mega.pytorch_b200/mega_core/_lib.py:

```python
import ctypes
import os

import torch

_HERE = os.path.dirname(os.path.abspath(__file__))
_PKG_ROOT = os.path.dirname(_HERE)
LIB_PATH = os.environ.get("MEGA_B200_LIB", os.path.join(_PKG_ROOT, "lib", "libmega_b200.so"))

if not os.path.exists(LIB_PATH):
    raise ImportError(
        "libmega_b200.so not found at %s -- run `python mega.pytorch_b200/build.py` "
        "(or __graft_entry__.build()) first; there is no fallback path" % LIB_PATH)

lib = ctypes.CDLL(LIB_PATH)

c_f32p = ctypes.c_void_p
c_ll = ctypes.c_longlong
c_int = ctypes.c_int


class ConvGemmDesc(ctypes.Structure):
    _fields_ = [
        ("a", c_f32p),
        ("a_n", c_int), ("a_h", c_int), ("a_w", c_int), ("a_c", c_int),
        ("a_stride_w", c_ll), ("a_stride_h", c_ll), ("a_stride_n", c_ll),
        ("b", c_f32p),
        ("b_n", c_int), ("b_k", c_int),
        ("b_stride_n", c_ll), ("b_stride_tap", c_ll),
        ("taps_r", c_int), ("taps_s", c_int), ("dil", c_int), ("pad", c_int),
        ("k_per_tap", c_int),
        ("out", c_f32p),
        ("out_ld", c_ll),
        ("n_img", c_int), ("out_h", c_int), ("out_w", c_int), ("cout", c_int),
        ("scale", c_f32p), ("bias", c_f32p), ("residual", c_f32p),
        ("res_ld", c_ll),
        ("relu", c_int),
        ("tile_h", c_int), ("tile_w", c_int), ("block_n", c_int),
        ("batch", c_int),
        ("a_c_off", c_int), ("a_n_off", c_int), ("b_k_off", c_int), ("b_n_off", c_int),
        ("out_c_off", c_int), ("out_n_off", c_int), ("res_c_off", c_int), ("res_n_off", c_int),
        ("bias_z_off", c_int),
        ("precision", c_int),
        ("max_ctas", c_int),
        ("stream_k", c_int),
        ("workspace", ctypes.c_void_p),
        ("workspace_bytes", c_ll),
        ("out_f16", c_int),
        ("pdl", c_int),
        ("stride_h", c_int), ("stride_w", c_int), ("pad_w_set", c_int), ("pad_w", c_int),
        ("out_stride_h", c_ll), ("out_stride_n", c_ll), ("res_stride_h", c_ll), ("res_stride_n", c_ll),
        ("b_lo_tap_off", c_int), ("res_split", c_int), ("acc_scale", ctypes.c_float), ("group_width", c_int),
    ]


lib.mega_last_error.restype = ctypes.c_char_p
lib.mega_abi_version.restype = c_int
lib.mega_device_ok.restype = c_int
lib.mega_conv_gemm.argtypes = [ctypes.POINTER(ConvGemmDesc), ctypes.c_void_p]
lib.mega_conv_gemm.restype = c_int
lib.mega_conv_gemm_tf32.argtypes = [ctypes.POINTER(ConvGemmDesc), ctypes.c_void_p]
lib.mega_conv_gemm_tf32.restype = c_int
lib.mega_conv_gemm_workspace_bytes.restype = c_ll
lib.mega_conv_chain_plan_bytes.argtypes = [c_int]
lib.mega_conv_chain_plan_bytes.restype = c_ll
lib.mega_conv_chain_encode.argtypes = [ctypes.POINTER(ConvGemmDesc), c_int, ctypes.c_void_p, c_ll, ctypes.POINTER(c_int)]
lib.mega_conv_chain_encode.restype = c_int
lib.mega_conv_chain_launch.argtypes = [ctypes.c_void_p, c_int, c_int, ctypes.c_void_p, ctypes.c_void_p, c_int]
lib.mega_conv_chain_launch.restype = c_int
lib.mega_conv_chain_encode2.argtypes = [ctypes.POINTER(ConvGemmDesc), c_int, ctypes.c_void_p, c_ll, ctypes.POINTER(c_int), c_int]
lib.mega_conv_chain_encode2.restype = c_int
lib.mega_conv_chain_launch2.argtypes = [ctypes.c_void_p, c_int, c_int, ctypes.c_void_p, ctypes.c_void_p, c_int, c_int]
lib.mega_conv_chain_launch2.restype = c_int
lib.mega_conv_chain_set_trace.argtypes = [ctypes.c_void_p, c_int]
lib.mega_conv_chain_set_trace.restype = c_int
lib.mega_conv_chain_set_trace2.argtypes = [ctypes.c_void_p, c_int, c_int]
lib.mega_conv_chain_set_trace2.restype = c_int
lib.mega_nms_host.argtypes = [ctypes.c_void_p, ctypes.c_void_p, c_int, ctypes.c_float, c_int, ctypes.c_void_p, ctypes.c_void_p]
lib.mega_nms_host.restype = c_int
lib.mega_roi_align_forward_nchw_host.argtypes = [ctypes.c_void_p, c_int, c_int, c_int, c_int, ctypes.c_void_p, c_int,
                                                 ctypes.c_float, c_int, c_int, c_int, c_int, ctypes.c_void_p]
lib.mega_roi_align_forward_nchw_host.restype = c_int
lib.mega_set_split3_seg_len.argtypes = [c_int]
lib.mega_set_split3_seg_len.restype = c_int
lib.mega_set_tf32_rounding.argtypes = [c_int]
lib.mega_set_tf32_rounding.restype = c_int


class MegaError(RuntimeError):
    pass


def check(status, what=""):
    if status != 0:
        msg = lib.mega_last_error().decode("utf-8", "replace")
        raise MegaError("%s failed (status %d): %s" % (what or "libmega_b200 call", status, msg))


def stream_ptr():
    return ctypes.c_void_p(torch.cuda.current_stream().cuda_stream)


def ptr(t):
    if t is None:
        return None
    return ctypes.c_void_p(t.data_ptr())


def require_cuda(*tensors):
    for t in tensors:
        if t is not None and not t.is_cuda:
            raise MegaError("libmega_b200 ops take CUDA tensors only (got a %s tensor); "
                            "the B200 path has no CPU fallback" % t.device)


_vp, _i, _f, _ll = ctypes.c_void_p, ctypes.c_int, ctypes.c_float, ctypes.c_longlong
lib.mega_nms_workspace_bytes.argtypes = [_i]
lib.mega_nms_workspace_bytes.restype = _ll
lib.mega_nms.argtypes = [_vp, _vp, _i, _f, _vp, _ll, _vp, _vp, _vp]
lib.mega_nms.restype = _i
lib.mega_rpn_select_workspace_bytes.argtypes = [_i, _i, _i, _i, _i]
lib.mega_rpn_select_workspace_bytes.restype = _ll
lib.mega_rpn_select.argtypes = [_vp, _ll, _i, _i, _i, _i, _i, _i, _vp, _f, _f, _i, _i, _f, _f, _vp, _ll, _vp, _vp,
                                _vp, _vp, _vp]
lib.mega_rpn_select.restype = _i
lib.mega_roi_align_forward_nchw.argtypes = [_vp, _i, _i, _i, _i, _vp, _i, _f, _i, _i, _i, _vp, _vp]
lib.mega_roi_align_forward_nchw.restype = _i
lib.mega_roi_align_forward_nhwc.argtypes = [_vp, _i, _i, _i, _ll, _vp, _i, _i, _vp, _i, _f, _i, _i, _i, _vp, _ll, _vp]
lib.mega_roi_align_forward_nhwc.restype = _i
lib.mega_roi_align_forward_nhwc_f16.argtypes = [_vp, _i, _i, _i, _ll, _vp, _i, _i, _vp, _i, _f, _i, _i, _i, _vp, _ll, _vp]
lib.mega_roi_align_forward_nhwc_split16.argtypes = [_vp, _i, _i, _i, _ll, _vp, _i, _i, _vp, _i, _f, _i, _i, _i, _vp, _ll, _vp]
lib.mega_roi_align_forward_nhwc_split16.restype = _i
lib.mega_roi_align_forward_nhwc_f16.restype = _i
lib.mega_stem_im2col_f16.argtypes = [_vp, _i, _i, _i, _i, _vp, _vp]
lib.mega_stem_im2col_f16.restype = _i
lib.mega_maxpool3x3s2_nhwc_f16.argtypes = [_vp, _i, _i, _i, _i, _vp, _vp]
lib.mega_maxpool3x3s2_nhwc_f16.restype = _i
lib.mega_relation_softmax_f16.argtypes = [_vp, _vp, _i, _i, _vp, _vp, _vp, _vp, _vp, _vp, _i, _vp, _i, _f, _vp]
lib.mega_relation_softmax_split16.argtypes = [_vp, _vp, _i, _i, _vp, _vp, _vp, _vp, _vp, _vp, _i, _vp, _i, _f, _vp]
lib.mega_relation_softmax_split16.restype = _i
lib.mega_relation_softmax_f16.restype = _i
lib.mega_relation_softmax_pe.argtypes = [_vp, _vp, _i, _i, _vp, _vp, _vp, _vp, _vp, _vp, _i, _vp, _i, _f, _vp]
lib.mega_relation_softmax_pe_split16.argtypes = [_vp, _vp, _i, _i, _vp, _vp, _vp, _vp, _vp, _vp, _i, _vp, _i, _f, _vp]
lib.mega_relation_softmax_pe_split16.restype = _i
lib.mega_relation_softmax_pe.restype = _i
lib.mega_fgfa_pool_image.argtypes = [_vp, _i, _i, _vp, _i, _vp]
lib.mega_fgfa_pool_image.restype = _i
lib.mega_fgfa_build_pairs.argtypes = [_vp, _ll, _vp, _i, _i, _i, _i, _vp, _i, _vp]
lib.mega_fgfa_build_pairs.restype = _i
lib.mega_avgpool2_nhwc.argtypes = [_vp, _i, _i, _i, _i, _ll, _vp, _ll, _i, _vp]
lib.mega_avgpool2_nhwc.restype = _i
lib.mega_fgfa_aggregate.argtypes = [_vp, _ll, _i, _i, _i, _vp, _i, _i, _vp, _i, _i, _i, _vp, _ll, _vp, _i, _vp]
lib.mega_fgfa_aggregate.restype = _i
lib.mega_stem_prep.argtypes = [_vp, _i, _i, _i, _i, _vp, _i, _vp]
lib.mega_stem_prep.restype = _i
lib.mega_stem_im2col.argtypes = [_vp, _i, _i, _i, _i, _vp, _vp]
lib.mega_stem_im2col.restype = _i
lib.mega_maxpool3x3s2_nhwc.argtypes = [_vp, _i, _i, _i, _i, _vp, _vp]
lib.mega_maxpool3x3s2_nhwc.restype = _i
lib.mega_gather_rows.argtypes = [_vp, _ll, _vp, _i, _i, _vp, _ll, _vp]
lib.mega_gather_rows.restype = _i
lib.mega_copy_rows.argtypes = [_vp, _ll, _vp, _vp, _ll, _vp, _i, _i, _vp]
lib.mega_copy_rows.restype = _i
class CopyJob(ctypes.Structure):
    _fields_ = [("src", ctypes.c_void_p), ("src_ld", ctypes.c_longlong), ("src_idx", ctypes.c_void_p),
                ("dst", ctypes.c_void_p), ("dst_ld", ctypes.c_longlong), ("dst_idx", ctypes.c_void_p),
                ("n_rows", ctypes.c_int), ("row_len", ctypes.c_int)]


lib.mega_copy_rows_batch.argtypes = [ctypes.POINTER(CopyJob), _i, _vp]
lib.mega_copy_rows_batch.restype = _i
lib.mega_split16_pack.argtypes = [_vp, _vp, _ll, _vp]
lib.mega_split16_pack.restype = _i
lib.mega_split16_unpack.argtypes = [_vp, _vp, _ll, _vp]
lib.mega_split16_unpack.restype = _i
lib.mega_transpose_2d.argtypes = [_vp, _i, _i, _i, _vp, _vp]
lib.mega_transpose_2d.restype = _i
lib.mega_relation_softmax.argtypes = [_vp, _i, _i, _vp, _vp, _vp, _vp, _vp, _vp, _i, _vp, _i, _f, _vp]
lib.mega_relation_softmax.restype = _i
lib.mega_box_postprocess_workspace_bytes.argtypes = [_i, _i]
lib.mega_box_postprocess_workspace_bytes.restype = _ll
lib.mega_box_postprocess.argtypes = [_vp, _i, _vp, _i, _vp, _vp, _i, _i, _f, _f, _f, _f, _i, _f, _f, _f, _f, _vp, _ll,
                                     _vp, _vp, _vp, _i, _vp, _vp]
lib.mega_box_postprocess.restype = _i

lib.mega_sigmoid_focalloss_forward.argtypes = [_vp, _vp, _i, _i, _f, _f, _vp, _vp]
lib.mega_sigmoid_focalloss_forward.restype = _i
lib.mega_sigmoid_focalloss_backward.argtypes = [_vp, _vp, _vp, _i, _i, _f, _f, _vp, _vp]
lib.mega_sigmoid_focalloss_backward.restype = _i
lib.mega_deform_im2col.argtypes = [_vp, _vp, _vp] + [_i] * 14 + [_vp, _vp]
lib.mega_deform_im2col.restype = _i
lib.mega_deform_psroi_pooling_forward.argtypes = [_vp, _vp, _vp, _i, _i, _i, _i, _i, _f, _i, _i, _i, _i, _i, _f, _i, _vp,
                                                  _vp, _vp]
lib.mega_deform_psroi_pooling_forward.restype = _i

lib.mega_roi_align_backward_nchw.argtypes = [_vp, _vp, _i, _f, _i, _i, _i, _i, _i, _i, _i, _vp, _vp]
lib.mega_roi_align_backward_nchw.restype = _i
lib.mega_roi_pool_forward.argtypes = [_vp, _vp, _i, _f, _i, _i, _i, _i, _i, _vp, _vp, _vp]
lib.mega_roi_pool_forward.restype = _i
lib.mega_roi_pool_backward.argtypes = [_vp, _vp, _vp, _i, _i, _i, _i, _i, _i, _vp, _vp]
lib.mega_roi_pool_backward.restype = _i
lib.mega_deform_im2col_kq.argtypes = [_vp, _vp, _vp] + [_i] * 14 + [_vp, _vp]
lib.mega_deform_im2col_kq.restype = _i
lib.mega_deform_col2im_fused.argtypes = [_vp, _vp, _vp, _vp] + [_i] * 14 + [_vp, _vp, _vp, _vp]
lib.mega_deform_col2im_fused.restype = _i
lib.mega_channel_sum_nchw.argtypes = [_vp, _i, _i, _i, _vp, _vp]
lib.mega_channel_sum_nchw.restype = _i
lib.mega_deform_psroi_pooling_backward.argtypes = [_vp, _vp, _vp, _vp, _vp, _i, _i, _i, _i, _i, _f, _i, _i, _i, _i, _i,
                                                   _f, _i, _vp, _vp, _vp]
lib.mega_deform_psroi_pooling_backward.restype = _i
lib.mega_image_transform_u8.argtypes = [_vp, _i, _i, _ll, _ll, _ll, _vp, _vp, _i, _vp, _vp, _i, _i, _i, _vp, _vp, _i, _vp, _vp]
lib.mega_image_transform_u8.restype = _i
lib.mega_dff_warp_scale.argtypes = [_vp, _i, _i, _vp, _i, _vp, _ll, _i, _i, _vp, _ll, _i, _vp]
lib.mega_dff_warp_scale.restype = _i
lib.mega_vid_match_host.argtypes = [_vp, _i, _vp, _vp, _i, _f, ctypes.c_double, _vp, _vp]
lib.mega_vid_match_host.restype = _i
lib.mega_seq_nms_workspace_bytes.argtypes = [_i, _i, _i]
lib.mega_seq_nms_workspace_bytes.restype = _ll
lib.mega_seq_nms.argtypes = [_vp, _vp, _vp, _vp, _i, _i, _vp, _i, _i, _f, _f, _i, _vp, _ll, _vp, _vp, _vp]
lib.mega_seq_nms.restype = _i
lib.mega_image_transform_u8_ex.argtypes = [_vp, _i, _i, _ll, _ll, _ll, _vp, _vp, _i, _vp, _vp, _i, _i, _i, _vp, _vp, _i, _i,
                                           _vp, _vp]
lib.mega_image_transform_u8_ex.restype = _i
lib.mega_bbox_aug_workspace_bytes.argtypes = [_i, _i, _i]
lib.mega_bbox_aug_workspace_bytes.restype = _ll
lib.mega_bbox_aug_collect.argtypes = [_vp, _i, _vp, _i, _vp, _vp, _i, _i, _i, _i, _i, _i, _i, ctypes.c_double,
                                      ctypes.c_double, _f, _f, _f, _f, _f, _vp, _ll, _vp]
lib.mega_bbox_aug_collect.restype = _i
lib.mega_bbox_aug_merge.argtypes = [_i, _i, _i, _f, _i, _vp, _ll, _vp, _vp, _vp, _i, _vp, _vp]
lib.mega_bbox_aug_merge.restype = _i

EXPORTS = [
    "mega_last_error", "mega_abi_version", "mega_device_ok", "mega_conv_gemm", "mega_conv_gemm_tf32", "mega_conv_gemm_workspace_bytes", "mega_set_tf32_rounding",
    "mega_conv_chain_plan_bytes", "mega_conv_chain_encode", "mega_conv_chain_launch", "mega_conv_chain_set_trace",
    "mega_conv_chain_encode2", "mega_conv_chain_launch2", "mega_set_split3_seg_len", "mega_conv_chain_set_trace2", "mega_nms_host", "mega_roi_align_forward_nchw_host",
    "mega_nms_workspace_bytes", "mega_nms", "mega_rpn_select_workspace_bytes", "mega_rpn_select",
    "mega_roi_align_forward_nchw", "mega_roi_align_forward_nhwc", "mega_stem_im2col", "mega_maxpool3x3s2_nhwc",
    "mega_gather_rows", "mega_copy_rows", "mega_copy_rows_batch", "mega_transpose_2d", "mega_relation_softmax", "mega_box_postprocess_workspace_bytes",
    "mega_box_postprocess", "mega_sigmoid_focalloss_forward", "mega_sigmoid_focalloss_backward",
    "mega_deform_im2col", "mega_deform_psroi_pooling_forward",
    "mega_roi_align_forward_nhwc_f16", "mega_stem_im2col_f16", "mega_maxpool3x3s2_nhwc_f16", "mega_relation_softmax_f16", "mega_relation_softmax_pe",
    "mega_stem_prep", "mega_fgfa_pool_image", "mega_fgfa_build_pairs", "mega_avgpool2_nhwc", "mega_fgfa_aggregate",
    "mega_roi_align_backward_nchw", "mega_roi_pool_forward", "mega_roi_pool_backward", "mega_deform_im2col_kq",
    "mega_deform_col2im_fused", "mega_channel_sum_nchw", "mega_deform_psroi_pooling_backward",
    "mega_image_transform_u8", "mega_dff_warp_scale", "mega_vid_match_host", "mega_split16_pack", "mega_split16_unpack", "mega_relation_softmax_split16", "mega_relation_softmax_pe_split16", "mega_roi_align_forward_nhwc_split16",
    "mega_seq_nms_workspace_bytes", "mega_seq_nms",
    "mega_image_transform_u8_ex", "mega_bbox_aug_workspace_bytes", "mega_bbox_aug_collect", "mega_bbox_aug_merge",
]
```

mega.pytorch_b200/mega_core/b200/ops.py:

```python
import ctypes
import math
import weakref

import torch

from .. import _lib
from .._lib import ConvGemmDesc, check, lib, ptr, require_cuda, stream_ptr


LAUNCHES = [0]


def _launch_conv_gemm(d):
    if _CHAIN_MODE[0] == "record":
        _CHAIN_REC[0].append(_copy_desc(d))
        return
    if _CHAIN_MODE[0] == "skip":
        return

    def run():
        check(lib.mega_conv_gemm(ctypes.byref(d), stream_ptr()), "mega_conv_gemm")
    _run_timed(run, _desc_flops(d), _desc_info(d))
    LAUNCHES[0] += 1


TIMING_HOOK = [None]


def _run_timed(run, flops, info):
    h = TIMING_HOOK[0]
    if h is None:
        run()
    else:
        h(run, flops, info)


def _desc_flops(d):
    return 2.0 * d.n_img * d.out_h * d.out_w * d.batch * d.cout * d.k_per_tap * d.taps_r * d.taps_s


def _desc_info(d):
    return {"m": d.n_img * d.out_h * d.out_w, "batch": d.batch, "cout": d.cout, "k": d.k_per_tap,
            "taps": d.taps_r * d.taps_s, "bn": d.block_n, "sk": d.stream_k, "res": bool(d.residual), "out16": d.out_f16,
            "precision": d.precision}


_CHAIN_MODE = [None]
_CHAIN_REC = [None]
CHAINS_ENABLED = [True]
MAX_BN = [256]


def _copy_desc(d):
    c = ConvGemmDesc()
    ctypes.memmove(ctypes.byref(c), ctypes.byref(d), ctypes.sizeof(ConvGemmDesc))
    return c


class ConvChain(object):
    def __init__(self, descs, device, max_ctas=0, depth=1):
        n = len(descs)
        self.n, self.depth = n, depth
        arr = (ConvGemmDesc * n)(*descs)
        nbytes = int(lib.mega_conv_chain_plan_bytes(n))
        host = torch.zeros(nbytes + 128, dtype=torch.uint8)
        off = (-host.data_ptr()) % 128
        grid = ctypes.c_int(0)
        check(lib.mega_conv_chain_encode2(arr, n, ctypes.c_void_p(host.data_ptr() + off), nbytes, ctypes.byref(grid), depth),
              "mega_conv_chain_encode2")
        if max_ctas > 0 and grid.value > max_ctas:
            raise _lib.MegaError("conv chain: a layer wants %d CTAs, more than max_ctas=%d (pass max_ctas to every "
                                 "conv_gemm of the chain)" % (grid.value, max_ctas))
        self.grid = grid.value
        dev_buf = torch.zeros(nbytes + 128, dtype=torch.uint8, device=device)
        doff = (-dev_buf.data_ptr()) % 128
        self.plan = dev_buf[doff:doff + nbytes]
        self.plan.copy_(host[off:off + nbytes])
        self._keep = dev_buf
        self.sync = torch.zeros(4, dtype=torch.int32, device=device)
        self.flops = sum(_desc_flops(d) for d in descs)
        self.info = {"chain_layers": n, "grid": self.grid, "depth": depth, "layers": [_desc_info(d) for d in descs]}
        torch.cuda.current_stream(device).synchronize()

    def launch(self):
        def run():
            check(lib.mega_conv_chain_launch2(ptr(self.plan), self.n, self.grid, ptr(self.sync), stream_ptr(),
                                              1 if PDL[0] else 0, self.depth), "mega_conv_chain_launch2")
        _run_timed(run, self.flops, self.info)
        LAUNCHES[0] += 1


class chain(object):

    def __init__(self, cache, key, device, enabled=True, max_ctas=0, interleave=False, depth=1):
        if SM_LIMIT[0] > 0 or WS_LANE[0] != 0:
            key = tuple(key) + ("sm", SM_LIMIT[0], WS_LANE[0])
        if SM_LIMIT[0] > 0:
            max_ctas = min(max_ctas, SM_LIMIT[0]) if max_ctas > 0 else SM_LIMIT[0]
        self.cache, self.key, self.device, self.max_ctas = cache, key, device, max_ctas
        self.enabled = enabled and CHAINS_ENABLED[0] and _CHAIN_MODE[0] is None
        self.interleave = interleave and self.enabled
        self.depth = depth
        self.split = None

    def next_lane(self):
        if self.enabled and _CHAIN_MODE[0] == "record":
            assert self.interleave and self.split is None
            self.split = len(_CHAIN_REC[0])

    def __enter__(self):
        if not self.enabled:
            return self
        self.saved_bn = MAX_BN[0]
        MAX_BN[0] = 128
        if self.key in self.cache:
            _CHAIN_MODE[0] = "skip"
        else:
            _CHAIN_MODE[0] = "record"
            _CHAIN_REC[0] = []
        return self

    def __exit__(self, et, ev, tb):
        if not self.enabled:
            return False
        mode = _CHAIN_MODE[0]
        _CHAIN_MODE[0] = None
        MAX_BN[0] = self.saved_bn
        if et is not None:
            _CHAIN_REC[0] = None
            return False
        if mode == "record":
            descs = _CHAIN_REC[0]
            _CHAIN_REC[0] = None
            depth = self.depth
            if self.interleave:
                assert self.split is not None and 2 * self.split == len(descs), \
                    "interleaved chain: the two lanes must record the same number of layers (%s / %d)" % (self.split, len(descs))
                descs = [d for pair in zip(descs[:self.split], descs[self.split:]) for d in pair]
                depth = 2
            self.cache[self.key] = ConvChain(descs, self.device, self.max_ctas, depth)
        self.cache[self.key].launch()
        return False


import os as _os
DUAL_CHAIN = [_os.environ.get("MEGA_B200_DUAL_CHAIN", "1") != "0"]
DUAL_MIN_IMAGES = 4

PDL = [True]

_gemm_ws = {}
WS_LANE = [0]
SM_LIMIT = [0]


class sm_limit(object):

    def __init__(self, n, lane=None):
        self.n, self.lane = int(n), lane

    def __enter__(self):
        self.saved = (SM_LIMIT[0], WS_LANE[0])
        SM_LIMIT[0] = self.n
        if self.lane is not None:
            WS_LANE[0] = self.lane
        return self

    def __exit__(self, *a):
        SM_LIMIT[0], WS_LANE[0] = self.saved
        return False


def gemm_workspace(device):
    key = (device, WS_LANE[0])
    ws = _gemm_ws.get(key)
    if ws is None:
        ws = torch.zeros(int(lib.mega_conv_gemm_workspace_bytes()), dtype=torch.uint8, device=device)
        _gemm_ws[key] = ws
    return ws


def pick_tile(h, w):
    best = None
    for tw in (128, 64, 32, 16, 8, 4, 2, 1):
        th = 128 // tw
        tiles = -(-h // th) * -(-w // tw)
        key = (tiles, -tw)
        if best is None or key < best[0]:
            best = (key, th, tw)
    return best[1], best[2]


PRECISION = [0]
PRECISION_NAMES = {"tf32": 0, "fp32x3": 1, "f16": 0}


class precision(object):

    def __init__(self, name):
        self.value = PRECISION_NAMES[name] if isinstance(name, str) else int(name)

    def __enter__(self):
        self.saved = PRECISION[0]
        PRECISION[0] = self.value

    def __exit__(self, *a):
        PRECISION[0] = self.saved
        return False


_PRESPLIT = {}


def presplit(w):
    assert w.is_cuda and w.dtype == torch.float32 and w.is_contiguous() and w.dim() in (2, 3)
    w3 = w if w.dim() == 3 else w.view(1, *w.shape)
    taps = w3.shape[0]
    combo = torch.empty(2 * taps, w3.shape[1], w3.shape[2], device=w.device, dtype=torch.float32)
    combo[:taps].copy_(w3)
    hi = (w3.view(torch.int32) & -8192).view(torch.float32)
    combo[taps:].copy_(w3 - hi)
    out = combo[:taps] if w.dim() == 3 else combo[0]
    _PRESPLIT[out.data_ptr()] = (weakref.ref(out), taps, tuple(w3.shape[1:]))
    return out


SPLIT16 = [_os.environ.get("MEGA_B200_SPLIT16", "1") != "0"]
SPLIT16_ATT = [_os.environ.get("MEGA_B200_SPLIT16_ATT", "1") != "0"]
_SPLIT16_BUFS = {}
_SPLIT16_W = {}


def mark_split16(t):
    assert t.dtype == torch.float32
    st = t.untyped_storage()
    _SPLIT16_BUFS[st.data_ptr()] = weakref.ref(st)
    return t


def unmark_split16(t):
    _SPLIT16_BUFS.pop(t.untyped_storage().data_ptr(), None)
    return t


def is_split16(t):
    if t is None or t.dtype != torch.float32:
        return False
    st = t.untyped_storage()
    r = _SPLIT16_BUFS.get(st.data_ptr())
    if r is None:
        return False
    if r() is None:
        del _SPLIT16_BUFS[st.data_ptr()]
        return False
    return True


def pack_split16(x, out=None):
    require_cuda(x, out)
    dst = x if out is None else out
    assert x.dtype == torch.float32 and x.is_contiguous() and dst.is_contiguous() and dst.numel() == x.numel()
    assert not is_split16(x) or out is not None, "already split-fp16"
    check(lib.mega_split16_pack(ptr(x), ptr(dst), x.numel(), stream_ptr()), "mega_split16_pack")
    return mark_split16(dst)


def unpack_split16(x, out):
    require_cuda(x, out)
    assert x.is_contiguous() and out.is_contiguous() and out.numel() == x.numel() and out.dtype == torch.float32
    check(lib.mega_split16_unpack(ptr(x), ptr(out), x.numel(), stream_ptr()), "mega_split16_unpack")
    return out


def split16_encode(x):
    assert x.dtype == torch.float32 and x.shape[-1] % 32 == 0
    xc = x.contiguous()
    hi = xc.clamp(-65504.0, 65504.0).half()
    lo = (xc - hi.float()).clamp(-65504.0, 65504.0).half()
    g = xc.shape[:-1] + (xc.shape[-1] // 32, 1, 32)
    both = torch.cat([hi.view(g), lo.view(g)], dim=-2)
    return both.reshape(xc.shape[:-1] + (2 * xc.shape[-1],)).view(torch.float32)


def split16_decode(p):
    h = p.contiguous().view(torch.float16)
    g = h.view(p.shape[:-1] + (p.shape[-1] // 32, 2, 32)).float()
    return (g[..., 0, :] + g[..., 1, :]).reshape(p.shape)


def pack_weights_split16(w, scale=None):
    assert w.dtype == torch.float32 and w.dim() in (2, 3) and w.shape[-1] % 32 == 0
    w0 = w
    if scale is not None:
        w = w * scale.to(w.device).float().view(-1, 1)
    m = float(w.abs().max())
    e = 0 if m == 0.0 else 13 - int(math.floor(math.log2(m)))
    e = max(-24, min(e, 40))
    gw = _grouped_width(w0)
    out = split16_encode(w * (2.0 ** e))
    _SPLIT16_W[out.data_ptr()] = (weakref.ref(out), 2.0 ** -e)
    if gw is not None:
        _GROUPED_W[out.data_ptr()] = (weakref.ref(out), gw)
    return out


def _split16_weight(w):
    r = _SPLIT16_W.get(w.data_ptr())
    if r is None:
        return None
    if r[0]() is None:
        del _SPLIT16_W[w.data_ptr()]
        return None
    return r[1]


def _split16_fmt(t):
    if t is None or t.dtype != torch.float32:
        return None
    s = _split16_weight(t)
    if s is not None:
        return s
    return 1.0 if is_split16(t) else None


TUNED = {}
AUTOTUNE = [False]
BLOCK_NS = (32, 64, 96, 128, 160, 192, 256)


def save_tuned(path):
    import json
    with open(path, "w") as fh:
        json.dump({"device": torch.cuda.get_device_name(0), "entries": [[list(k), list(v)] for k, v in TUNED.items()]}, fh)


def load_tuned(path):
    import json
    import os
    if not os.path.exists(path):
        return 0
    with open(path) as fh:
        data = json.load(fh)
    if torch.cuda.is_available() and data.get("device") != torch.cuda.get_device_name(0):
        return 0
    for k, v in data["entries"]:
        if len(k) == 22:
            k = list(k) + [0]
        TUNED.setdefault(tuple(bool(x) if isinstance(x, bool) else x for x in k), tuple(v))
    return len(data["entries"])


def _shape_key(d):
    return (d.a_n, d.a_h, d.a_w, d.a_c, d.a_stride_w, d.b_n, d.b_k, d.taps_r, d.taps_s, d.dil, d.k_per_tap, d.n_img,
            d.out_h, d.out_w, d.cout, d.tile_h, d.tile_w, d.batch, bool(d.residual), d.out_ld, d.out_c_off,
            d.precision, d.out_f16) + ((d.stride_h, d.stride_w) if (d.stride_h, d.stride_w) != (1, 1) else ())


def _candidates(cout, prec=0, out_f16=0):
    cands = []
    for bn in ((64, 128) if prec in (1, 3) else BLOCK_NS):
        if out_f16 and bn % 64:
            continue
        if bn > MAX_BN[0]:
            continue
        if bn >= 2 * cout and bn > (64 if out_f16 else 32):
            continue
        for sk in (0, 1):
            cands.append((bn, sk))
    return cands


def _autotune(d):
    best = None
    for bn, sk in _candidates(d.cout, d.precision, d.out_f16):
        d.block_n, d.stream_k = bn, sk
        try:
            for _ in range(2):
                check(lib.mega_conv_gemm(ctypes.byref(d), stream_ptr()), "mega_conv_gemm")
            e0, e1 = torch.cuda.Event(enable_timing=True), torch.cuda.Event(enable_timing=True)
            e0.record()
            for _ in range(8):
                check(lib.mega_conv_gemm(ctypes.byref(d), stream_ptr()), "mega_conv_gemm")
            e1.record()
            e1.synchronize()
            t = e0.elapsed_time(e1) / 8
        except _lib.MegaError:
            continue
        if best is None or t < best[0]:
            best = (t, bn, sk)
    return best


def _autotune_chain(d):
    best = None
    dev = torch.device("cuda", torch.cuda.current_device())
    for bn, sk in _candidates(d.cout, d.precision, d.out_f16):
        c = _copy_desc(d)
        c.block_n, c.stream_k = bn, sk
        try:
            ch = ConvChain([c], dev, max_ctas=d.max_ctas)
            hook, TIMING_HOOK[0] = TIMING_HOOK[0], None
            try:
                for _ in range(2):
                    ch.launch()
                e0, e1 = torch.cuda.Event(enable_timing=True), torch.cuda.Event(enable_timing=True)
                e0.record()
                for _ in range(8):
                    ch.launch()
                e1.record()
                e1.synchronize()
            finally:
                TIMING_HOOK[0] = hook
            LAUNCHES[0] -= 10
            t = e0.elapsed_time(e1) / 8
        except _lib.MegaError:
            continue
        if best is None or t < best[0]:
            best = (t, bn, sk)
    return best


def pick_config(cout, m_tiles, batch, kb_per_tile, out_f16=False):
    if kb_per_tile >= 48:
        for bn in (32, 64, 128):
            if cout <= bn and not (out_f16 and bn % 64):
                return bn, 1
        return min(256, MAX_BN[0]), 1
    best = None
    for bn in BLOCK_NS:
        if out_f16 and bn % 64:
            continue
        if bn > MAX_BN[0]:
            continue
        if bn >= 2 * cout and bn > (64 if out_f16 else 32):
            continue
        tiles = m_tiles * (-(-cout // bn)) * batch
        cost = (-(-tiles // 132)) * (128 + bn)
        if best is None or cost < best[0] or (cost == best[0] and bn > best[1]):
            best = (cost, bn)
    return best[1], 0


def pick_block_n(cout, m_tiles=0, batch=1):
    return pick_config(cout, max(m_tiles, 1), batch, 1)[0]


GROUP_CHUNK = 64
GROUP_WIDTHS = (8, 16, 32, 64)
GROUP_DIAG = [True]
_GROUPED_W = {}


def _grouped_width(w):
    r = _GROUPED_W.get(w.data_ptr())
    if r is None:
        return None
    if r[0]() is None:
        del _GROUPED_W[w.data_ptr()]
        return None
    return r[1]


def pack_grouped_conv(w, groups, dev, dtype=torch.float32):
    c, gw, kh, kw = w.shape
    assert c == gw * groups and gw in GROUP_WIDTHS and c % GROUP_CHUNK == 0, \
        "grouped conv: %d channels in %d groups (group width must be one of %s, channels a multiple of %d)" % (
            c, groups, GROUP_WIDTHS, GROUP_CHUNK)
    taps = w.permute(2, 3, 0, 1).reshape(kh * kw, c, gw)
    out = torch.zeros(kh * kw, c, GROUP_CHUNK, dtype=w.dtype, device=w.device)
    col = torch.arange(c, device=w.device) % GROUP_CHUNK // gw * gw
    idx = (col.view(1, c, 1) + torch.arange(gw, device=w.device).view(1, 1, gw)).expand(kh * kw, c, gw)
    out.scatter_(2, idx, taps)
    out = out.contiguous().to(dev).to(dtype)
    _GROUPED_W[out.data_ptr()] = (weakref.ref(out), gw)
    return out


def grouped_fields(w):
    c, z = w.shape[1], GROUP_CHUNK
    return dict(batch=c // z, cout=z, k=z, block_n=z, a_c_off=z, b_n_off=z, out_c_off=z, res_c_off=z, bias_z_off=z)


def conv_gemm(a, w, out, *, taps=(1, 1), dil=1, pad=0, scale=None, bias=None, residual=None,
              relu=False, tile=None, block_n=None, cout=None, k=None, batch=1, a_c_off=0,
              a_n_off=0, b_k_off=0, b_n_off=0, out_c_off=0, out_n_off=0, res_c_off=0, res_n_off=0, bias_z_off=0,
              max_ctas=0, stream_k=None, out_hw=None, n_img=None, stride=(1, 1), pad_w=None, groups=1):
    if groups > 1:
        assert batch == 1 and cout is None and k is None and block_n is None and w.shape[2] == GROUP_CHUNK, \
            "conv_gemm(groups=...): pass the weight from pack_grouped_conv and no batched fields"
        g = grouped_fields(w)
        return conv_gemm(a, w, out, taps=taps, dil=dil, pad=pad, scale=scale, bias=bias, residual=residual, relu=relu,
                         tile=tile, max_ctas=max_ctas, stream_k=stream_k, out_hw=out_hw, n_img=n_img, stride=stride,
                         pad_w=pad_w, **g)
    require_cuda(a, w, out, scale, bias, residual)
    f16 = a.dtype == torch.float16
    assert a.dtype == w.dtype and a.dtype in (torch.float32, torch.float16), (a.dtype, w.dtype)
    assert out.dtype == torch.float32 or (f16 and out.dtype == torch.float16), (a.dtype, out.dtype)
    assert residual is None or residual.dtype == out.dtype
    out_f16 = out.dtype == torch.float16
    assert a.dim() == 4 and w.dim() == 3 and out.dim() == 4
    assert a.stride(3) == 1 and w.stride(2) == 1 and out.stride(3) == 1
    n, h, wd, c = a.shape
    t, rows, kk = w.shape
    assert t == taps[0] * taps[1]
    on, oh, ow, oc = out.shape
    if out_hw is not None:
        oh, ow = out_hw
    d = ConvGemmDesc()
    d.a = ptr(a)
    d.a_n, d.a_h, d.a_w, d.a_c = n, h, wd, c
    d.a_stride_w, d.a_stride_h, d.a_stride_n = a.stride(2), a.stride(1), a.stride(0)
    d.b = ptr(w)
    d.b_n, d.b_k = rows, kk
    d.b_stride_n, d.b_stride_tap = w.stride(1), w.stride(0)
    d.taps_r, d.taps_s, d.dil, d.pad = taps[0], taps[1], dil, pad
    d.k_per_tap = k if k is not None else kk
    d.out = ptr(out)
    d.out_ld = out.stride(2)
    d.n_img, d.out_h, d.out_w = (on if n_img is None else n_img), oh, ow
    d.cout = cout if cout is not None else rows
    d.scale, d.bias, d.residual = ptr(scale), ptr(bias), ptr(residual)
    d.res_ld = residual.stride(-2) if residual is not None else 0
    if oh > 1:
        d.out_stride_h = out.stride(1)
    if d.n_img > 1 or batch > 1:
        d.out_stride_n = out.stride(0)
    if residual is not None and residual.dim() == 4:
        if oh > 1:
            d.res_stride_h = residual.stride(1)
        if d.n_img > 1 or batch > 1:
            d.res_stride_n = residual.stride(0)
    d.relu = 2 if relu == "leaky" else (1 if relu else 0)
    d.stride_h, d.stride_w = stride
    if pad_w is not None:
        d.pad_w_set, d.pad_w = 1, pad_w
    th, tw = tile if tile is not None else pick_tile(oh, ow)
    d.tile_h, d.tile_w = th, tw
    m_tiles = d.n_img * (-(-oh // th)) * (-(-ow // tw))
    d.batch = batch
    kb_per_tile = taps[0] * taps[1] * (-(-d.k_per_tap // (64 if f16 else 32)))
    d.precision = 2 if f16 else PRECISION[0]
    d.out_f16 = 1 if out_f16 else 0
    fa, fb = _split16_fmt(a), _split16_fmt(w)
    if fa is not None or fb is not None:
        assert fa is not None and fb is not None, \
            "conv_gemm: both operands must be split-fp16 (ops.pack_split16 / pack_weights_split16) or neither (A %s, B %s)" % (
                "split" if fa is not None else "plain", "split" if fb is not None else "plain")
        assert scale is None, "conv_gemm: split-fp16 contractions take no scale (fold it: pack_weights_split16(w, scale))"
        d.precision = 3
        d.out_f16 = 1 if is_split16(out) else 0
        d.res_split = 1 if is_split16(residual) else 0
        d.acc_scale = fa * fb
    else:
        assert not (is_split16(out) or is_split16(residual)), \
            "conv_gemm: split-fp16 output / residual need split-fp16 operands"
    d.pdl = 1 if PDL[0] else 0
    auto_bn, auto_sk = pick_config(d.cout, m_tiles, batch, kb_per_tile, out_f16)
    if d.precision in (1, 3):
        auto_bn = 64 if d.cout <= 64 else 128
        if block_n not in (None, 64, 128):
            block_n = auto_bn
    d.block_n = block_n if block_n is not None else auto_bn
    d.stream_k = auto_sk if stream_k is None else int(stream_k)
    d.a_c_off, d.a_n_off, d.b_k_off, d.b_n_off = a_c_off, a_n_off, b_k_off, b_n_off
    d.out_c_off, d.out_n_off, d.res_c_off, d.res_n_off = out_c_off, out_n_off, res_c_off, res_n_off
    d.bias_z_off = bias_z_off
    gw = _grouped_width(w)
    if (gw is not None and GROUP_DIAG[0] and batch > 1 and d.cout == d.k_per_tap == d.block_n == GROUP_CHUNK
            and a_c_off == b_n_off == out_c_off == GROUP_CHUNK and b_k_off == 0):
        d.group_width = gw
    d.max_ctas = max_ctas
    if SM_LIMIT[0] > 0:
        d.max_ctas = min(max_ctas, SM_LIMIT[0]) if max_ctas > 0 else SM_LIMIT[0]
    if d.precision == 1 and batch == 1:
        ps = _PRESPLIT.get(w.data_ptr())
        if ps is not None and ps[0]() is None:
            del _PRESPLIT[w.data_ptr()]
            ps = None
        if ps is not None and ps[1] == t and ps[2] == (rows, kk) and w.stride(1) == kk:
            d.b_lo_tap_off = t
            d.b_stride_tap = rows * kk
    ws = gemm_workspace(a.device)
    d.workspace = ptr(ws)
    d.workspace_bytes = ws.numel()
    if block_n is None and stream_k is None:
        key = _shape_key(d) + ((MAX_BN[0],) if MAX_BN[0] != 256 else ())
        cfg = TUNED.get(key)
        aliased = residual is not None and residual.data_ptr() == out.data_ptr()
        if (cfg is None and AUTOTUNE[0] and not aliased and _CHAIN_MODE[0] != "skip"
                and not torch.cuda.is_current_stream_capturing()):
            best = _autotune_chain(d) if _CHAIN_MODE[0] == "record" else _autotune(d)
            if best is not None:
                cfg = TUNED[key] = (best[1], best[2], best[0])
        if cfg is not None:
            d.block_n, d.stream_k = cfg[0], cfg[1]
    _launch_conv_gemm(d)
    return out


def linear(x, w, out, *, bias=None, relu=False, residual=None, block_n=None, max_ctas=0, stream_k=None):
    m, kdim = x.shape
    nrows = w.shape[0]
    a4 = x.as_strided((1, 1, m, kdim), (x.stride(0) * m, x.stride(0) * m, x.stride(0), 1))
    o4 = out.as_strided((1, 1, m, out.shape[1]), (out.stride(0) * m, out.stride(0) * m, out.stride(0), 1))
    r4 = None
    if residual is not None:
        r4 = residual.as_strided((1, 1, m, residual.shape[1]),
                                 (residual.stride(0) * m, residual.stride(0) * m, residual.stride(0), 1))
    w3 = w.as_strided((1, nrows, kdim), (w.stride(0) * nrows, w.stride(0), 1))
    return conv_gemm(a4, w3, o4, bias=bias, relu=relu, residual=r4, tile=(1, 128), cout=nrows, block_n=block_n,
                     max_ctas=max_ctas, stream_k=stream_k)


_ws_cache = {}


def _workspace(key, nbytes, device):
    ws = _ws_cache.get((key, device))
    if ws is None or ws.numel() < nbytes:
        ws = torch.empty(int(nbytes), dtype=torch.uint8, device=device)
        _ws_cache[(key, device)] = ws
    return ws


def nms_device(boxes, scores, thresh, keep=None, count=None):
    require_cuda(boxes, scores)
    n = boxes.shape[0]
    boxes = boxes.contiguous().float()
    scores = scores.contiguous().float()
    if keep is None:
        keep = torch.empty(max(n, 1), dtype=torch.int64, device=boxes.device)
    if count is None:
        count = torch.zeros(1, dtype=torch.int32, device=boxes.device)
    nbytes = lib.mega_nms_workspace_bytes(n)
    if nbytes < 0:
        raise _lib.MegaError("nms: n=%d exceeds the single-pass capacity (8192 boxes)" % n)
    ws = _workspace("nms", max(nbytes, 256), boxes.device)
    check(lib.mega_nms(ptr(boxes), ptr(scores), n, float(thresh), ptr(ws), ws.numel(), ptr(keep), ptr(count),
                       stream_ptr()), "mega_nms")
    LAUNCHES[0] += 4
    return keep, count


def rpn_select(head, n_img, h, w, base_anchors, im_w, im_h, pre_nms, post_nms, nms_thresh, min_size=0.0,
               stride=16, out=None, want_anchor=False):
    require_cuda(head, base_anchors)
    a = base_anchors.shape[0]
    ld = head.shape[-1]
    dev = head.device
    if out is None:
        boxes = torch.empty(n_img, post_nms, 4, device=dev)
        scores = torch.empty(n_img, post_nms, device=dev)
        count = torch.empty(n_img, dtype=torch.int32, device=dev)
        anchor = torch.empty(n_img, post_nms, dtype=torch.int32, device=dev) if want_anchor else None
    else:
        boxes, scores, anchor, count = out
    nbytes = lib.mega_rpn_select_workspace_bytes(n_img, h, w, a, pre_nms)
    if nbytes < 0:
        raise _lib.MegaError("rpn_select: pre_nms_top_n=%d exceeds 8192" % pre_nms)
    ws = _workspace("rpn%d" % n_img, nbytes, dev)
    check(lib.mega_rpn_select(ptr(head), head.stride(0), ld, n_img, h, w, a, stride, ptr(base_anchors), float(im_w),
                              float(im_h), pre_nms, post_nms, float(nms_thresh), float(min_size), ptr(ws), ws.numel(),
                              ptr(boxes), ptr(scores), ptr(anchor), ptr(count), stream_ptr()), "mega_rpn_select")
    LAUNCHES[0] += 4
    return boxes, scores, anchor, count


def roi_align_nchw(inp, rois, scale, ph, pw, sampling_ratio, out=None):
    require_cuda(inp, rois)
    inp = inp.contiguous().float()
    rois = rois.contiguous().float()
    n, c, h, w = inp.shape
    k = rois.shape[0]
    if out is None:
        out = torch.empty(k, c, ph, pw, device=inp.device)
    check(lib.mega_roi_align_forward_nchw(ptr(inp), n, c, h, w, ptr(rois), k, float(scale), ph, pw, sampling_ratio,
                                          ptr(out), stream_ptr()), "mega_roi_align_forward_nchw")
    LAUNCHES[0] += 1
    return out


def roi_align_nhwc(feat, boxes, roi_batch, scale, ph, pw, sampling_ratio, out):
    require_cuda(feat, boxes, roi_batch, out)
    n, h, w, c = feat.shape
    k = boxes.shape[0]
    assert out.dtype == feat.dtype
    fn = lib.mega_roi_align_forward_nhwc_f16 if feat.dtype == torch.float16 else lib.mega_roi_align_forward_nhwc
    if is_split16(feat):
        if h <= 64 and w <= 64 and c % 128 == 0 and ph <= 7 and pw <= 7:
            fn = lib.mega_roi_align_forward_nhwc_split16
            mark_split16(out)
        else:
            plain = unpack_split16(feat.contiguous(), torch.empty_like(feat))
            unmark_split16(out)
            roi_align_nhwc(plain, boxes, roi_batch, scale, ph, pw, sampling_ratio, out)
            return pack_split16(out)
    else:
        unmark_split16(out)
    check(fn(ptr(feat), c, h, w, feat.stride(0), ptr(boxes), boxes.stride(0), 0,
                                          ptr(roi_batch), k, float(scale), ph, pw, sampling_ratio, ptr(out),
                                          out.stride(0), stream_ptr()), "mega_roi_align_forward_nhwc")
    LAUNCHES[0] += 1
    return out


def stem_im2col(img, out, kpad=160):
    require_cuda(img, out)
    n, c, h, w = img.shape
    assert c == 3 and img.is_contiguous() and img.dtype == torch.float32
    fn = lib.mega_stem_im2col_f16 if out.dtype == torch.float16 else lib.mega_stem_im2col
    check(fn(ptr(img), n, h, w, kpad, ptr(out), stream_ptr()), "mega_stem_im2col")
    LAUNCHES[0] += 1
    return out


def stem_prep(img, out):
    require_cuda(img, out)
    n, c, h, w = img.shape
    assert c == 3 and img.is_contiguous() and img.dtype == torch.float32 and out.shape[1] == h + 6 and out.shape[3] == 8
    check(lib.mega_stem_prep(ptr(img), n, h, w, out.shape[2], ptr(out), 1 if out.dtype == torch.float16 else 0,
                             stream_ptr()), "mega_stem_prep")
    LAUNCHES[0] += 1
    return out


def maxpool3x3s2(x, out):
    require_cuda(x, out)
    n, h, w, c = x.shape
    assert x.dtype == out.dtype
    fn = lib.mega_maxpool3x3s2_nhwc_f16 if x.dtype == torch.float16 else lib.mega_maxpool3x3s2_nhwc
    check(fn(ptr(x), n, h, w, c, ptr(out), stream_ptr()), "mega_maxpool3x3s2_nhwc")
    LAUNCHES[0] += 1
    return out


def _as_f32_rows(t):
    return t.view(torch.float32) if t.dtype == torch.float16 else t


def gather_rows(src, idx, dst, n_rows=None, row_len=None):
    require_cuda(src, idx, dst)
    assert idx.dtype == torch.int32 and src.dtype == dst.dtype
    if src.dtype == torch.float16:
        assert row_len is None
        src, dst = _as_f32_rows(src), _as_f32_rows(dst)
    n_rows = idx.numel() if n_rows is None else n_rows
    row_len = src.shape[-1] if row_len is None else row_len
    if copy_batch.active[0] is not None:
        copy_batch.active[0].append(_copy_job(src, idx, dst, None, n_rows, row_len))
        return dst
    check(lib.mega_gather_rows(ptr(src), src.stride(-2), ptr(idx), n_rows, row_len, ptr(dst), dst.stride(-2),
                               stream_ptr()), "mega_gather_rows")
    LAUNCHES[0] += 1
    return dst


def copy_rows(src, dst, n_rows, row_len=None, src_idx=None, dst_idx=None):
    require_cuda(src, dst, src_idx, dst_idx)
    assert src.dtype == dst.dtype
    if src.dtype == torch.float16:
        assert row_len is None
        src, dst = _as_f32_rows(src), _as_f32_rows(dst)
    row_len = src.shape[-1] if row_len is None else row_len
    if copy_batch.active[0] is not None:
        copy_batch.active[0].append(_copy_job(src, src_idx, dst, dst_idx, n_rows, row_len))
        return dst
    check(lib.mega_copy_rows(ptr(src), src.stride(-2), ptr(src_idx), ptr(dst), dst.stride(-2), ptr(dst_idx), n_rows,
                             row_len, stream_ptr()), "mega_copy_rows")
    LAUNCHES[0] += 1
    return dst


class copy_batch(object):
    active = [None]

    def __enter__(self):
        copy_batch.active[0] = []
        return self

    def __exit__(self, et, ev, tb):
        jobs, copy_batch.active[0] = copy_batch.active[0], None
        if et is not None or not jobs:
            return False
        for i in range(0, len(jobs), 16):
            part = jobs[i:i + 16]
            arr = (_lib.CopyJob * len(part))(*part)
            check(lib.mega_copy_rows_batch(arr, len(part), stream_ptr()), "mega_copy_rows_batch")
            LAUNCHES[0] += 1
        return False


def _copy_job(src, src_idx, dst, dst_idx, n_rows, row_len):
    j = _lib.CopyJob()
    j.src, j.src_ld, j.src_idx = src.data_ptr(), src.stride(-2), (src_idx.data_ptr() if src_idx is not None else None)
    j.dst, j.dst_ld, j.dst_idx = dst.data_ptr(), dst.stride(-2), (dst_idx.data_ptr() if dst_idx is not None else None)
    j.n_rows, j.row_len = n_rows, row_len
    return j


def transpose_2d(x, out, n_img, rows, cols):
    require_cuda(x, out)
    check(lib.mega_transpose_2d(ptr(x), n_img, rows, cols, ptr(out), stream_ptr()), "mega_transpose_2d")
    LAUNCHES[0] += 1
    return out


def relation_softmax(logits, n_rows, ldm, scale, boxes_q=None, boxes_k=None, wg=None, bg=None, dim_mat=None,
                     m_valid=None, m_host=0, n_valid=None, n_valid_off=0, probs_f16=None, host_w=None):
    split = probs_f16 is not None and probs_f16.dtype == torch.float32
    if split:
        assert is_split16(probs_f16) and probs_f16.numel() == logits.numel() and ldm % 32 == 0
    if host_w is not None and boxes_q is not None:
        require_cuda(logits, boxes_q, boxes_k, m_valid, n_valid, probs_f16)
        wg_h, bg_h, dim_h = host_w
        assert not wg_h.is_cuda and wg_h.dtype == torch.float32 and wg_h.is_contiguous() and wg_h.numel() == 1024
        assert probs_f16 is None or split or probs_f16.dtype == torch.float16
        fn = lib.mega_relation_softmax_pe_split16 if split else lib.mega_relation_softmax_pe
        check(fn(ptr(logits), ptr(probs_f16), n_rows, ldm, ptr(boxes_q), ptr(boxes_k),
                                           ptr(wg_h), ptr(bg_h), ptr(dim_h), ptr(m_valid), m_host, ptr(n_valid),
                                           n_valid_off, float(scale), stream_ptr()), "mega_relation_softmax_pe")
        LAUNCHES[0] += 1
        return logits
    require_cuda(logits, boxes_q, boxes_k, wg, bg, dim_mat, m_valid, n_valid, probs_f16)
    if probs_f16 is not None:
        assert split or probs_f16.dtype == torch.float16
        fn = lib.mega_relation_softmax_split16 if split else lib.mega_relation_softmax_f16
        check(fn(ptr(logits), ptr(probs_f16), n_rows, ldm, ptr(boxes_q), ptr(boxes_k),
                                            ptr(wg), ptr(bg), ptr(dim_mat), ptr(m_valid), m_host, ptr(n_valid),
                                            n_valid_off, float(scale), stream_ptr()), "mega_relation_softmax_f16")
    else:
        check(lib.mega_relation_softmax(ptr(logits), n_rows, ldm, ptr(boxes_q), ptr(boxes_k), ptr(wg), ptr(bg),
                                        ptr(dim_mat), ptr(m_valid), m_host, ptr(n_valid), n_valid_off, float(scale),
                                        stream_ptr()), "mega_relation_softmax")
    LAUNCHES[0] += 1
    return logits


def box_postprocess(logits, deltas, proposals, count, num_classes, im_w, im_h, score_thresh, nms_thresh, max_det,
                    weights, out):
    require_cuda(logits, deltas, proposals, count)
    r = proposals.shape[0]
    nbytes = lib.mega_box_postprocess_workspace_bytes(r, num_classes)
    if nbytes < 0:
        raise _lib.MegaError("box_postprocess: at most 512 proposals per image")
    ws = _workspace("post", nbytes, logits.device)
    ob, os_, ol, oc = out
    check(lib.mega_box_postprocess(ptr(logits), logits.stride(0), ptr(deltas), deltas.stride(0), ptr(proposals),
                                   ptr(count), r, num_classes, float(im_w), float(im_h), float(score_thresh),
                                   float(nms_thresh), max_det, *[float(x) for x in weights], ptr(ws), ws.numel(),
                                   ptr(ob), ptr(os_), ptr(ol), ob.shape[0], ptr(oc), stream_ptr()),
          "mega_box_postprocess")
    LAUNCHES[0] += 2
    return out


def bbox_aug_workspace_bytes(num_passes, r_max, num_classes):
    nbytes = lib.mega_bbox_aug_workspace_bytes(num_passes, r_max, num_classes)
    if nbytes < 0:
        raise _lib.MegaError("bbox_aug: %d passes x %d proposals = %d merged rows per class, %d classes: out of range "
                             "(at most 8192 merged rows, at least 2 classes)"
                             % (num_passes, r_max, num_passes * r_max, num_classes))
    return nbytes


def bbox_aug_collect(logits, deltas, proposals, count, num_classes, pass_index, num_passes, im_w, im_h, hflip, ratio_w,
                     ratio_h, score_thresh, weights, workspace):
    require_cuda(logits, deltas, proposals, count, workspace)
    r = proposals.shape[0]
    check(lib.mega_bbox_aug_collect(ptr(logits), logits.stride(0), ptr(deltas), deltas.stride(0), ptr(proposals),
                                    ptr(count), r, num_classes, pass_index, num_passes, int(im_w), int(im_h),
                                    int(bool(hflip)), float(ratio_w), float(ratio_h), float(score_thresh),
                                    *[float(x) for x in weights], ptr(workspace), workspace.numel(), stream_ptr()),
          "mega_bbox_aug_collect")
    LAUNCHES[0] += 1


def bbox_aug_merge(num_passes, r_max, num_classes, nms_thresh, max_det, workspace, out):
    require_cuda(workspace, *out)
    ob, os_, ol, oc = out
    check(lib.mega_bbox_aug_merge(num_passes, r_max, num_classes, float(nms_thresh), int(max_det), ptr(workspace),
                                  workspace.numel(), ptr(ob), ptr(os_), ptr(ol), ob.shape[0], ptr(oc), stream_ptr()),
          "mega_bbox_aug_merge")
    LAUNCHES[0] += 2
    return out


SEQ_NMS_RESCORE = {"avg": 0, "max": 1}


def seq_nms_workspace_bytes(num_frames, max_det, num_classes):
    nbytes = lib.mega_seq_nms_workspace_bytes(num_frames, max_det, num_classes)
    if nbytes < 0:
        raise _lib.MegaError("seq_nms: %d frames of at most %d detections, %d classes: out of range (max_det <= 512)"
                             % (num_frames, max_det, num_classes))
    return nbytes


def seq_nms(boxes, scores, labels, counts, video_offsets, num_classes, link_iou=0.5, nms_iou=0.3, rescore="avg"):
    require_cuda(boxes, scores, labels, counts, video_offsets)
    if rescore not in SEQ_NMS_RESCORE:
        raise ValueError("seq_nms: rescore must be one of %s, got %r" % (sorted(SEQ_NMS_RESCORE), rescore))
    f, d = scores.shape
    boxes = boxes.contiguous().float()
    scores = scores.contiguous().float()
    labels = labels.contiguous().int()
    counts = counts.contiguous().int()
    video_offsets = video_offsets.contiguous().int()
    nbytes = seq_nms_workspace_bytes(f, d, num_classes)
    ws = _workspace("seq_nms", nbytes, boxes.device)
    out_scores = torch.empty(f, d, dtype=torch.float32, device=boxes.device)
    keep = torch.empty(f, d, dtype=torch.uint8, device=boxes.device)
    check(lib.mega_seq_nms(ptr(boxes), ptr(scores), ptr(labels), ptr(counts), f, d, ptr(video_offsets),
                           video_offsets.numel() - 1, int(num_classes), float(link_iou), float(nms_iou),
                           SEQ_NMS_RESCORE[rescore], ptr(ws), ws.numel(), ptr(out_scores), ptr(keep), stream_ptr()),
          "mega_seq_nms")
    LAUNCHES[0] += 3
    return out_scores, keep


def _is16(t):
    return 1 if t.dtype == torch.float16 else 0


def fgfa_pool_image(img, out):
    require_cuda(img, out)
    h, w = img.shape[-2:]
    assert img.dtype == torch.float32 and img.is_contiguous()
    check(lib.mega_fgfa_pool_image(ptr(img), h, w, ptr(out), _is16(out), stream_ptr()), "mega_fgfa_pool_image")
    LAUNCHES[0] += 1
    return out


def fgfa_build_pairs(ring, slots, key_pos, pairs):
    require_cuda(ring, slots, pairs)
    s, hq, wq, _ = ring.shape
    assert ring.dtype == pairs.dtype and slots.dtype == torch.int32
    check(lib.mega_fgfa_build_pairs(ptr(ring), ring.stride(0), ptr(slots), slots.numel(), key_pos, hq, wq, ptr(pairs),
                                    _is16(ring), stream_ptr()), "mega_fgfa_build_pairs")
    LAUNCHES[0] += 1
    return pairs


def avgpool2_nhwc(x, out):
    require_cuda(x, out)
    n, h, w, c = x.shape
    assert x.dtype == out.dtype and x.stride(3) == 1 and out.stride(3) == 1
    check(lib.mega_avgpool2_nhwc(ptr(x), n, h, w, c, x.stride(2), ptr(out), out.stride(2), _is16(x), stream_ptr()),
          "mega_avgpool2_nhwc")
    LAUNCHES[0] += 1
    return out


def fgfa_aggregate(ring, slots, key_pos, flow, out, feat_channels, embed_channels, weights_out=None):
    require_cuda(ring, slots, flow, out, weights_out)
    s, h, w, ld = ring.shape
    assert flow.dtype == torch.float32 and ring.dtype == out.dtype
    check(lib.mega_fgfa_aggregate(ptr(ring), ring.stride(0), ld, feat_channels, embed_channels, ptr(slots), slots.numel(),
                                  key_pos, ptr(flow), flow.stride(2), h, w, ptr(out), out.stride(-2), ptr(weights_out),
                                  _is16(ring), stream_ptr()), "mega_fgfa_aggregate")
    LAUNCHES[0] += 1
    return out


def dff_warp_scale(key_feats, flow, scale, out):
    require_cuda(key_feats, flow, scale, out)
    h, w, c = key_feats.shape
    assert flow.dtype == torch.float32 and key_feats.dtype == scale.dtype == out.dtype
    assert key_feats.stride(2) == 1 and scale.stride(2) == 1 and out.stride(2) == 1 and key_feats.stride(0) == w * key_feats.stride(1)
    check(lib.mega_dff_warp_scale(ptr(key_feats), key_feats.stride(1), c, ptr(flow), flow.stride(1), ptr(scale),
                                  scale.stride(1), h, w, ptr(out), out.stride(1), _is16(key_feats), stream_ptr()),
          "mega_dff_warp_scale")
    LAUNCHES[0] += 1
    return out
```

Before: 143.0.

## Pair CTAs in 2-CTA clusters sharing A tiles via TMA multicast for f16x3 conv GEMM

After: 145.5 (median of 6 runs). 1.7% higher.

```diff
diff --git a/include/mega_b200.h b/include/mega_b200.h
--- a/include/mega_b200.h
+++ b/include/mega_b200.h
@@ -57,6 +57,7 @@
 int mega_conv_gemm(const mega_conv_gemm_desc* desc, void* stream);
 int mega_conv_gemm_tf32(const mega_conv_gemm_desc* desc, void* stream);
 long long mega_conv_gemm_workspace_bytes(void);
+int mega_conv_gemm_clustered(const mega_conv_gemm_desc* desc);
 
 long long mega_conv_chain_plan_bytes(int n_layers);
 int mega_conv_chain_encode(const mega_conv_gemm_desc* descs, int n_layers, void* plan_host, long long plan_bytes,
diff --git a/mega.pytorch_b200/csrc/common.cuh b/mega.pytorch_b200/csrc/common.cuh
--- a/mega.pytorch_b200/csrc/common.cuh
+++ b/mega.pytorch_b200/csrc/common.cuh
@@ -66,6 +66,16 @@
 }
 __device__ __forceinline__ void mbar_arrive(uint64_t* bar) {
   asm volatile("mbarrier.arrive.shared::cta.b64 _, [%0];" ::"r"(smem_u32(bar)) : "memory");
+}
+__device__ __forceinline__ void mbar_arrive_cluster(uint64_t* bar, uint32_t cta_rank) {
+  asm volatile(
+      "{\n"
+      ".reg .b32 ra;\n"
+      "mapa.shared::cluster.u32 ra, %0, %1;\n"
+      "mbarrier.arrive.shared::cluster.b64 _, [ra];\n"
+      "}\n" ::"r"(smem_u32(bar)),
+      "r"(cta_rank)
+      : "memory");
 }
 __device__ __forceinline__ bool mbar_try_wait(uint64_t* bar, uint32_t parity) {
   uint32_t ok;
@@ -126,6 +136,19 @@
       : "memory");
 }
 
+__device__ __forceinline__ void tma_load_4d_multicast(void* dst, const CUtensorMap* tm, uint64_t* bar, uint16_t cta_mask,
+                                                      int c0, int c1, int c2, int c3) {
+  asm volatile(
+      "cp.async.bulk.tensor.4d.shared::cluster.global.tile.mbarrier::complete_tx::bytes.multicast::cluster"
+      " [%0], [%1, {%4, %5, %6, %7}], [%2], %3;" ::"r"(smem_u32(dst)),
+      "l"(tm), "r"(smem_u32(bar)), "h"(cta_mask), "r"(c0), "r"(c1), "r"(c2), "r"(c3)
+      : "memory");
+}
+
+__device__ __forceinline__ void cluster_sync() {
+  asm volatile("barrier.cluster.arrive.release;\nbarrier.cluster.wait.acquire;" ::: "memory");
+}
+
 __device__ __forceinline__ void tma_store_4d(const CUtensorMap* tm, const void* src, int c0, int c1, int c2, int c3) {
   asm volatile(
       "cp.async.bulk.tensor.4d.global.shared::cta.bulk_group [%0, {%2, %3, %4, %5}], [%1];" ::"l"(tm),
diff --git a/mega.pytorch_b200/csrc/conv_gemm.cu b/mega.pytorch_b200/csrc/conv_gemm.cu
--- a/mega.pytorch_b200/csrc/conv_gemm.cu
+++ b/mega.pytorch_b200/csrc/conv_gemm.cu
@@ -52,6 +52,36 @@
 }
 
 namespace mega {
+
+static int encode_a_map(const mega_conv_gemm_desc* d, CUtensorMap* tm, int halves) {
+  EncodeTiledFn enc = get_encode_fn();
+  if (!enc) {
+    mega_set_error("conv_gemm: cuTensorMapEncodeTiled unavailable (no CUDA driver?)");
+    return MEGA_ERR_CUDA;
+  }
+  const bool f16 = d->precision == kModeF16;
+  const int esz = f16 ? 2 : 4;
+  const int stride_h = d->stride_h > 0 ? d->stride_h : 1, stride_w = d->stride_w > 0 ? d->stride_w : 1;
+  const int th = d->tile_h / halves, tw = d->tile_w;
+  const CUtensorMapDataType dt = f16 ? CU_TENSOR_MAP_DATA_TYPE_FLOAT16
+                                     : (g_tf32_round && d->precision == kModeTf32) ? CU_TENSOR_MAP_DATA_TYPE_TFLOAT32
+                                                                                    : CU_TENSOR_MAP_DATA_TYPE_FLOAT32;
+  cuuint64_t gdim[4] = {static_cast<cuuint64_t>(d->a_c), static_cast<cuuint64_t>(d->a_w),
+                        static_cast<cuuint64_t>(d->a_h), static_cast<cuuint64_t>(d->a_n)};
+  cuuint64_t gstr[3] = {static_cast<cuuint64_t>(d->a_stride_w) * esz, static_cast<cuuint64_t>(d->a_stride_h) * esz,
+                        static_cast<cuuint64_t>(d->a_stride_n) * esz};
+  cuuint32_t box[4] = {static_cast<cuuint32_t>(mode_bk(d->precision)), static_cast<cuuint32_t>((tw - 1) * stride_w + 1),
+                       static_cast<cuuint32_t>((th - 1) * stride_h + 1), 1};
+  cuuint32_t estr[4] = {1, static_cast<cuuint32_t>(stride_w), static_cast<cuuint32_t>(stride_h), 1};
+  CUresult r = enc(tm, dt, 4, const_cast<void*>(d->a), gdim, gstr, box, estr, CU_TENSOR_MAP_INTERLEAVE_NONE,
+                   CU_TENSOR_MAP_SWIZZLE_128B, CU_TENSOR_MAP_L2_PROMOTION_L2_256B, CU_TENSOR_MAP_FLOAT_OOB_FILL_NONE);
+  if (r != CUDA_SUCCESS) {
+    mega_set_error("conv_gemm: encode A tensor map failed (CUresult %d) dims %d %d %d %d strides %lld %lld %lld",
+                   static_cast<int>(r), d->a_c, d->a_w, d->a_h, d->a_n, d->a_stride_w, d->a_stride_h, d->a_stride_n);
+    return MEGA_ERR_CUDA;
+  }
+  return MEGA_OK;
+}
 
 int encode_conv_gemm_problem(const mega_conv_gemm_desc* d, CUtensorMap* tmA_p, CUtensorMap* tmB_p, CUtensorMap* tmOut_p,
                              CUtensorMap* tmRes_p, ConvGemmParams* p_out, int* ctas_out) {
@@ -138,26 +168,9 @@
                                                                  : CU_TENSOR_MAP_DATA_TYPE_FLOAT32;
   const CUtensorMapDataType odt = out16 ? CU_TENSOR_MAP_DATA_TYPE_FLOAT16 : CU_TENSOR_MAP_DATA_TYPE_FLOAT32;
 
-  CUtensorMap& tmA = *tmA_p;
   CUtensorMap& tmB = *tmB_p;
-  {
-    cuuint64_t gdim[4] = {static_cast<cuuint64_t>(d->a_c), static_cast<cuuint64_t>(d->a_w),
-                          static_cast<cuuint64_t>(d->a_h), static_cast<cuuint64_t>(d->a_n)};
-    cuuint64_t gstr[3] = {static_cast<cuuint64_t>(d->a_stride_w) * esz, static_cast<cuuint64_t>(d->a_stride_h) * esz,
-                          static_cast<cuuint64_t>(d->a_stride_n) * esz};
-    cuuint32_t box[4] = {static_cast<cuuint32_t>(bk), static_cast<cuuint32_t>((d->tile_w - 1) * stride_w + 1),
-                         static_cast<cuuint32_t>((d->tile_h - 1) * stride_h + 1), 1};
-    cuuint32_t estr[4] = {1, static_cast<cuuint32_t>(stride_w), static_cast<cuuint32_t>(stride_h), 1};
-    CUresult r = enc(&tmA, dt, 4, const_cast<void*>(d->a), gdim, gstr, box, estr, CU_TENSOR_MAP_INTERLEAVE_NONE,
-                     CU_TENSOR_MAP_SWIZZLE_128B, CU_TENSOR_MAP_L2_PROMOTION_L2_256B,
-                     CU_TENSOR_MAP_FLOAT_OOB_FILL_NONE);
-    if (r != CUDA_SUCCESS) {
-      mega_set_error("conv_gemm: encode A tensor map failed (CUresult %d) dims %d %d %d %d strides %lld %lld %lld",
-                     static_cast<int>(r), d->a_c, d->a_w, d->a_h, d->a_n, d->a_stride_w, d->a_stride_h,
-                     d->a_stride_n);
-      return MEGA_ERR_CUDA;
-    }
-  }
+  const int erc = encode_a_map(d, tmA_p, 1);
+  if (erc != MEGA_OK) return erc;
   {
     const int taps = d->taps_r * d->taps_s;
     MEGA_ARG_CHECK(d->b_lo_tap_off == 0 || (strict && d->b_lo_tap_off == taps && d->batch == 1),
@@ -273,6 +286,7 @@
   p.total_units = tiles * p.kb_per_tile;
   p.total_tiles = tiles;
   p.stream_k = d->stream_k ? 1 : 0;
+  p.cluster = 1;
   p.seg_len = g_seg_len;
   p.b_lo_tap_off = d->b_lo_tap_off;
   p.res_split = d->res_split ? 1 : 0;
@@ -307,6 +321,31 @@
   return MEGA_OK;
 }
 
+static bool clustered(const mega_conv_gemm_desc* d) {
+  return d->precision == kModeF16x3 && d->group_width == 0 && d->block_n > 0 && mega_ceil_div(d->cout, d->block_n) % 2 == 0 &&
+         d->tile_h > 1 && d->max_ctas != 1;
+}
+static bool make_clustered(const mega_conv_gemm_desc* d, CUtensorMap* tmA, ConvGemmParams* p, int* clusters_out, int* erc) {
+  *erc = MEGA_OK;
+  if (!clustered(d)) return false;
+  *erc = encode_a_map(d, tmA, 2);
+  if (*erc != MEGA_OK) return false;
+  p->cluster = 2;
+  p->total_tiles /= 2;
+  p->total_units = p->total_tiles * p->kb_per_tile;
+  const long long pairs = p->total_tiles;
+  long long clusters = p->stream_k ? p->total_units / kMinUnits : pairs;
+  if (clusters < 1) clusters = 1;
+  if (clusters > g_num_sms / 2) clusters = g_num_sms / 2;
+  if (d->max_ctas > 0 && clusters > d->max_ctas / 2) clusters = d->max_ctas / 2;
+  if (p->stream_k && p->kb_per_tile >= 256 && pairs <= clusters) {
+    const long long aligned = (clusters / pairs) * pairs;
+    if (aligned * 100 >= clusters * 85) clusters = aligned;
+  }
+  *clusters_out = static_cast<int>(clusters);
+  return true;
+}
+
 }
 
 extern "C" int mega_conv_gemm(const mega_conv_gemm_desc* d, void* stream_v) {
@@ -314,8 +353,9 @@
   CUtensorMap tmA, tmB, tmOut, tmRes;
   ConvGemmParams p;
   int ctas = 0;
-  const int erc = encode_conv_gemm_problem(d, &tmA, &tmB, &tmOut, &tmRes, &p, &ctas);
+  int erc = encode_conv_gemm_problem(d, &tmA, &tmB, &tmOut, &tmRes, &p, &ctas);
   if (erc != MEGA_OK) return erc;
+  if (!make_clustered(d, &tmA, &p, &ctas, &erc) && erc != MEGA_OK) return erc;
   const bool out16 = d->out_f16 != 0;
   dim3 grid(static_cast<unsigned>(ctas), 1, 1);
   const int pdl = d->pdl ? 1 : 0;
@@ -328,4 +368,6 @@
   }
 }
 
+extern "C" int mega_conv_gemm_clustered(const mega_conv_gemm_desc* d) { return d != nullptr && clustered(d) ? 1 : 0; }
+
 extern "C" int mega_conv_gemm_tf32(const mega_conv_gemm_desc* d, void* stream) { return mega_conv_gemm(d, stream); }
diff --git a/mega.pytorch_b200/csrc/conv_gemm_kernel.cuh b/mega.pytorch_b200/csrc/conv_gemm_kernel.cuh
--- a/mega.pytorch_b200/csrc/conv_gemm_kernel.cuh
+++ b/mega.pytorch_b200/csrc/conv_gemm_kernel.cuh
@@ -50,6 +50,7 @@
   long long total_units;
   long long total_tiles;
   int stream_k;
+  int cluster;
   float* part_ws;
   int* counters;
   int seg_len;
@@ -135,6 +136,10 @@
   }
 };
 
+__device__ __forceinline__ int item_tile(const ConvGemmParams& p, int item, int cs, int rank) {
+  return (cs * (item / p.m_tiles) + rank) * p.m_tiles + item % p.m_tiles;
+}
+
 template <int THREADS>
 __device__ __forceinline__ void epi_bar_sync() { asm volatile("bar.sync 1, %0;" ::"n"(THREADS) : "memory"); }
 
@@ -155,12 +160,12 @@
 }
 
 template <int THREADS>
-__device__ __forceinline__ bool sk_elect_finisher(const ConvGemmParams& p, int U, int grid, int KB, int t, int epi_tid,
-                                                  int* flag, int& c_first, int& c_last) {
+__device__ __forceinline__ bool sk_elect_finisher(const ConvGemmParams& p, int U, int grid, int KB, int item, int t,
+                                                  int epi_tid, int* flag, int& c_first, int& c_last) {
   __threadfence();
   epi_bar_sync<THREADS>();
-  c_first = unit_owner(U, grid, t * KB);
-  c_last = unit_owner(U, grid, t * KB + KB - 1);
+  c_first = unit_owner(U, grid, item * KB);
+  c_last = unit_owner(U, grid, item * KB + KB - 1);
   if (epi_tid == 0) {
     const int parts = c_last - c_first + 1;
     const int old = atomicAdd(&p.counters[t], 1);
@@ -173,20 +178,29 @@
   if (finisher) __threadfence();
   return finisher;
 }
-
-__device__ __forceinline__ void sk_reduce(const ConvGemmParams& p, int U, int grid, int KB, int t, int c_first, int c_last,
-                                          int row, int bn, int col0, float (&acc)[32]) {
+template <int THREADS>
+__device__ __forceinline__ bool sk_elect_finisher(const ConvGemmParams& p, int U, int grid, int KB, int t, int epi_tid,
+                                                  int* flag, int& c_first, int& c_last) {
+  return sk_elect_finisher<THREADS>(p, U, grid, KB, t, t, epi_tid, flag, c_first, c_last);
+}
+
+__device__ __forceinline__ void sk_reduce(const ConvGemmParams& p, int U, int grid, int KB, int item, int c_first,
+                                          int c_last, int cs, int rank, int row, int bn, int col0, float (&acc)[32]) {
 #pragma unroll
   for (int j = 0; j < 32; ++j) acc[j] = 0.f;
   for (int oc = c_first; oc <= c_last; ++oc) {
-    const int slot = (cta_first_unit(U, grid, oc) >= t * KB) ? 0 : 1;
-    const float* ws = sk_part_row(p, oc, slot, row, bn) + col0;
+    const int slot = (cta_first_unit(U, grid, oc) >= item * KB) ? 0 : 1;
+    const float* ws = sk_part_row(p, oc * cs + rank, slot, row, bn) + col0;
 #pragma unroll
     for (int j = 0; j < 32; j += 4) {
       const float4 v = __ldcg(reinterpret_cast<const float4*>(ws + j));
       acc[j] += v.x; acc[j + 1] += v.y; acc[j + 2] += v.z; acc[j + 3] += v.w;
     }
   }
+}
+__device__ __forceinline__ void sk_reduce(const ConvGemmParams& p, int U, int grid, int KB, int t, int c_first, int c_last,
+                                          int row, int bn, int col0, float (&acc)[32]) {
+  sk_reduce(p, U, grid, KB, t, c_first, c_last, 1, 0, row, bn, col0, acc);
 }
 
 struct StoreBox {
@@ -233,7 +247,8 @@
 __device__ __forceinline__ void produce_pass(const CUtensorMap* tmA, const CUtensorMap* tmB, uint64_t* full_bar,
                                              uint64_t* empty_bar, PipeState& ps, uint8_t* stage0, int stage_bytes, int b_off,
                                              int b_lo_off, int bk, uint32_t tx_bytes, const ConvGemmParams& p,
-                                             const TileCoord& tc, int n0, int kb0, int kb1, int lane, F&& on_stage) {
+                                             const TileCoord& tc, int n0, int kb0, int kb1, int lane, F&& on_stage,
+                                             uint16_t mc_mask = 0, int a_off = 0, int a_dh = 0) {
   const int k_chunks = p.k_chunks, taps_s = p.taps_s;
   int tap = kb0 / k_chunks;
   int kc = kb0 - tap * k_chunks;
@@ -247,8 +262,13 @@
     uint8_t* dst = stage0 + ps.stage * stage_bytes;
     if (lane == 0) {
       mbar_arrive_expect_tx(&full_bar[ps.stage], tx_bytes);
-      tma_load_4d(dst, tmA, &full_bar[ps.stage], kc * bk + a_c0, tc.w0 * p.stride_w + sx * p.dil - p.pad_w,
-                  tc.h0 * p.stride_h + r * p.dil - p.pad, a_n);
+      if (mc_mask != 0)
+        tma_load_4d_multicast(dst + a_off, tmA, &full_bar[ps.stage], mc_mask, kc * bk + a_c0,
+                              tc.w0 * p.stride_w + sx * p.dil - p.pad_w,
+                              (tc.h0 + a_dh) * p.stride_h + r * p.dil - p.pad, a_n);
+      else
+        tma_load_4d(dst, tmA, &full_bar[ps.stage], kc * bk + a_c0, tc.w0 * p.stride_w + sx * p.dil - p.pad_w,
+                    tc.h0 * p.stride_h + r * p.dil - p.pad, a_n);
     } else {
       tma_load_3d(dst + b_off, tmB, &full_bar[ps.stage], kc * bk + b_k0, b_n, tap);
       if (b_lo_off != 0) tma_load_3d(dst + b_lo_off, tmB, &full_bar[ps.stage], kc * bk + b_k0, b_n, tap + p.b_lo_tap_off);
@@ -441,7 +461,7 @@
 template <int PN, int STAGES, int MODE, class L, int GW = 0>
 __device__ __forceinline__ void mma_pass(uint8_t* smem, uint64_t* full_bar, uint64_t* empty_bar, uint64_t* split_bar,
                                          uint8_t* ring, uint64_t* ring_full, uint64_t* ring_empty, MmaState& ms, int kb0,
-                                         int kb1, int seg_len, int wg, int wtid, int hpc) {
+                                         int kb1, int seg_len, int wg, int wtid, int hpc, int peer = -1) {
   static_assert(GW == 0 || PN == 64, "grouped k-blocks need a 64-column pass");
   constexpr bool SPLIT3 = MODE == kModeSplit3;
   constexpr bool SEG = SPLIT3 || MODE == kModeF16x3;
@@ -471,7 +491,10 @@
       if (SPLIT3) wgmma_wait<0>(); else wgmma_wait<1>();
       if (pending >= 0) {
         __syncwarp();
-        if (lane == 0) mbar_arrive(&empty_bar[pending]);
+        if (lane == 0) {
+          mbar_arrive(&empty_bar[pending]);
+          if (peer >= 0) mbar_arrive_cluster(&empty_bar[pending], peer);
+        }
       }
       pending = ms.stage;
       if (++ms.stage == STAGES) {
@@ -483,7 +506,10 @@
     wgmma_wait_regs(d);
     if (pending >= 0) {
       __syncwarp();
-      if (lane == 0) mbar_arrive(&empty_bar[pending]);
+      if (lane == 0) {
+        mbar_arrive(&empty_bar[pending]);
+        if (peer >= 0) mbar_arrive_cluster(&empty_bar[pending], peer);
+      }
     }
     if constexpr (MODE == kModeF16x3) {
 #pragma unroll
@@ -549,7 +575,7 @@
   if (warp == 1 && lane == 0) {
     for (int s = 0; s < STAGES; ++s) {
       mbar_init(&full_bar[s], 1);
-      mbar_init(&empty_bar[s], 8);
+      mbar_init(&empty_bar[s], (PK && GW == 0) ? 8 * p.cluster : 8);
       mbar_init(&split_bar[s], 4);
     }
     for (int b = 0; b < kRingSlots; ++b) {
@@ -560,40 +586,53 @@
     fence_barrier_init();
   }
   __syncthreads();
+  const bool clustered = PK && GW == 0 && p.cluster == 2;
+  if (clustered) cluster_sync();
+  auto cluster_exit = [&]() {
+    if (clustered) cluster_sync();
+  };
   griddep_wait();
   griddep_launch_dependents();
   if (warp == 0) {
     if (PK) setmaxnreg_dec<kF16x3RegsProducer>();
     if (lane < 2) {
       PipeState ps = {0, 0};
-      WorkIter it(p, PK ? ctaid_x_here() : cta, grid);
-      int t;
+      const int me = PK ? ctaid_x_here() : cta;
+      const int cl = (PK && GW == 0) ? p.cluster - 1 : 0;
+      const int rank = me & cl;
+      WorkIter it(p, me >> cl, grid >> cl);
+      int item;
       int kb0, kb1;
       const bool b_lo = SPLIT3 && p.b_lo_tap_off > 0;
-      while (it.next(t, kb0, kb1)) {
-        const TileCoord tc = decode_tile(p, t, BN);
+      while (it.next(item, kb0, kb1)) {
+        const TileCoord tc = decode_tile(p, PK ? item_tile(p, item, cl + 1, rank) : item, BN);
         for (int pass = 0; pass < (BN > pass_n(BN) ? 2 : 1); ++pass)
           produce_pass<STAGES>(&tmA, &tmB, full_bar, empty_bar, ps, smem, L::kStageBytes, L::kABytes,
                                b_lo ? L::kABytes + L::kBBytes : 0, kBK, L::kHalf + (b_lo ? L::kBBytes : 0), p, tc,
-                               tc.n0 + pass * pass_n(BN), kb0, kb1, lane, [](int) {});
-      }
-    }
+                               tc.n0 + pass * pass_n(BN), kb0, kb1, lane, [](int) {}, cl ? 3 : 0,
+                               rank * (L::kABytes / 2), rank * (p.tile_h >> 1));
+      }
+    }
+    cluster_exit();
   } else if (warp >= kMmaWarp0) {
     if (PK) setmaxnreg_inc<kF16x3RegsMma>();
     const int wg = (warp - kMmaWarp0) >> 2;
     const int wtid = threadIdx.x - (kMmaWarp0 + 4 * wg) * 32;
     constexpr int P0 = pass_n(BN), P1 = BN - P0;
     MmaState ms = {0, 0, {0, 0}};
-    WorkIter it(p, PK ? ctaid_x_here() : cta, grid);
+    const int me = PK ? ctaid_x_here() : cta;
+    const int cl = (PK && GW == 0) ? p.cluster - 1 : 0;
+    WorkIter it(p, me >> cl, grid >> cl);
     int t;
     int kb0, kb1;
     while (it.next(t, kb0, kb1)) {
       mma_pass<P0, STAGES, MODE, L, GW>(smem, full_bar, empty_bar, split_bar, ring, ring_full, ring_empty, ms, kb0, kb1,
-                                        kSegLen, wg, wtid, 0);
+                                        kSegLen, wg, wtid, 0, cl ? (ctaid_x_here() & 1) ^ 1 : -1);
       if constexpr (P1 > 0)
         mma_pass<P1, STAGES, MODE, L>(smem, full_bar, empty_bar, split_bar, ring, ring_full, ring_empty, ms, kb0, kb1,
                                       kSegLen, wg, wtid, 0);
     }
+    cluster_exit();
   } else if (warp >= 6 && warp < 10 && !PK) {
     if (SPLIT3) {
       const int stid = threadIdx.x - kThreads;
@@ -641,15 +680,18 @@
     float* bias_s = reinterpret_cast<float*>(smem + L::kSbOffset);
     uint32_t rphase = 0;
     const int cta_e = ctaid_x_here();
-    WorkIter it(p, cta_e, grid);
-    int t;
+    const int cl = GW == 0 ? p.cluster - 1 : 0;
+    auto rank_here = [&]() { return ctaid_x_here() & cl; };
+    auto tile_of = [&](int i) { return cl ? item_tile(p, i, 2, rank_here()) : i; };
+    WorkIter it(p, cta_e >> cl, grid >> cl);
+    int item;
     int kb0, kb1;
     uint32_t seq0 = 0;
     const uint32_t sw = static_cast<uint32_t>(lane & 7);
     const bool res_split = p.res_split != 0;
     const float slope = p.relu == 2 ? 0.1f : 0.f;
-    for (int tile_item = 0; it.next(t, kb0, kb1); ++tile_item, seq0 += BN / 32) {
-      const TileCoord tc = decode_tile(p, t, BN);
+    for (int tile_item = 0; it.next(item, kb0, kb1); ++tile_item, seq0 += BN / 32) {
+      const TileCoord tc = decode_tile(p, tile_of(item), BN);
       const bool complete = (kb0 == 0 && kb1 == KB);
       const StoreBox box = store_box(p, tc, q);
       const int nchunks = min(BN / 32, (p.cout - tc.n0 + 31) / 32);
@@ -669,7 +711,7 @@
         int t2, k0, k1;
         has_next = peek.next(t2, k0, k1);
         if (has_next && epi_tid < BN) {
-          const TileCoord tc2 = decode_tile(p, t2, BN);
+          const TileCoord tc2 = decode_tile(p, tile_of(t2), BN);
           const int n = tc2.n0 + epi_tid;
           next_bias = (p.bias && n < p.cout) ? __ldg(p.bias + tc2.batch * p.bias_z_off + n) : 0.f;
         }
@@ -705,7 +747,7 @@
           ring_take(ring, ring_full, ring_empty, seq0 + j, row, raw);
           sk_publish(part, j * 32, raw);
         }
-        finalize = sk_elect_finisher<128>(p, U, grid, KB, t, epi_tid, epi_flag, c_first, c_last);
+        finalize = sk_elect_finisher<128>(p, U, it.grid, KB, item, tile_of(item), epi_tid, epi_flag, c_first, c_last);
         if (finalize) issue_residual();
       }
       if (finalize) {
@@ -715,7 +757,7 @@
           if (j < nchunks) {
             float acc[32];
             if (complete) load_chunk(j, acc);
-            else sk_reduce(p, U, grid, KB, t, c_first, c_last, row, BN, j * 32, acc);
+            else sk_reduce(p, U, it.grid, KB, item, c_first, c_last, cl + 1, rank_here(), row, BN, j * 32, acc);
             uint8_t* rowp = stage_buf + j * 4096 + lane * 128;
             const float4* biv = reinterpret_cast<const float4*>(bias_s + bsel * BN + j * 32);
 #pragma unroll
@@ -787,8 +829,10 @@
       if (has_next && epi_tid < BN) bias_s[(bsel ^ 1) * BN + epi_tid] = next_bias;
     }
     if (lane == 0) tma_store_wait<0>();
+    cluster_exit();
   } else if (PK) {
     setmaxnreg_dec<kF16x3RegsProducer>();
+    cluster_exit();
   } else if (warp >= 2 && warp < 6) {
     const int q = warp & 3;
     const int row = q * 32 + lane;
@@ -949,11 +993,28 @@
   cfg.blockDim = dim3(conv_gemm_threads(MODE), 1, 1);
   cfg.dynamicSmemBytes = L::kTotal;
   cfg.stream = stream;
-  cudaLaunchAttribute attr[1];
+  cudaLaunchAttribute attr[2];
   attr[0].id = cudaLaunchAttributeProgrammaticStreamSerialization;
   attr[0].val.programmaticStreamSerializationAllowed = 1;
   cfg.attrs = attr;
   cfg.numAttrs = pdl ? 1 : 0;
+  if (MODE == kModeF16x3 && GW == 0 && p.cluster == 2) {
+    attr[cfg.numAttrs].id = cudaLaunchAttributeClusterDimension;
+    attr[cfg.numAttrs].val.clusterDim.x = 2;
+    attr[cfg.numAttrs].val.clusterDim.y = 1;
+    attr[cfg.numAttrs].val.clusterDim.z = 1;
+    ++cfg.numAttrs;
+    static int max_clusters = 0;
+    if (max_clusters == 0) {
+      cfg.gridDim = dim3(2 * kMaxCtas, 1, 1);
+      MEGA_CUDA_CHECK(cudaOccupancyMaxActiveClusters(&max_clusters, conv_gemm_kernel<BN, STAGES, MODE, OUT16, GW>, &cfg));
+      if (max_clusters < 1) {
+        mega_set_error("conv_gemm: no 2-CTA cluster of this kernel fits on the device");
+        return MEGA_ERR_CUDA;
+      }
+    }
+    cfg.gridDim = dim3(2 * static_cast<unsigned>(grid.x < static_cast<unsigned>(max_clusters) ? grid.x : max_clusters), 1, 1);
+  }
   MEGA_CUDA_CHECK(cudaLaunchKernelEx(&cfg, conv_gemm_kernel<BN, STAGES, MODE, OUT16, GW>, tmA, tmB, tmOut, tmRes, p));
   return MEGA_OK;
 }
diff --git a/mega.pytorch_b200/mega_core/_lib.py b/mega.pytorch_b200/mega_core/_lib.py
--- a/mega.pytorch_b200/mega_core/_lib.py
+++ b/mega.pytorch_b200/mega_core/_lib.py
@@ -61,6 +61,8 @@
 lib.mega_conv_gemm_tf32.argtypes = [ctypes.POINTER(ConvGemmDesc), ctypes.c_void_p]
 lib.mega_conv_gemm_tf32.restype = c_int
 lib.mega_conv_gemm_workspace_bytes.restype = c_ll
+lib.mega_conv_gemm_clustered.argtypes = [ctypes.POINTER(ConvGemmDesc)]
+lib.mega_conv_gemm_clustered.restype = c_int
 lib.mega_conv_chain_plan_bytes.argtypes = [c_int]
 lib.mega_conv_chain_plan_bytes.restype = c_ll
 lib.mega_conv_chain_encode.argtypes = [ctypes.POINTER(ConvGemmDesc), c_int, ctypes.c_void_p, c_ll, ctypes.POINTER(c_int)]
@@ -230,7 +232,7 @@
 lib.mega_bbox_aug_merge.restype = _i
 
 EXPORTS = [
-    "mega_last_error", "mega_abi_version", "mega_device_ok", "mega_conv_gemm", "mega_conv_gemm_tf32", "mega_conv_gemm_workspace_bytes", "mega_set_tf32_rounding",
+    "mega_last_error", "mega_abi_version", "mega_device_ok", "mega_conv_gemm", "mega_conv_gemm_tf32", "mega_conv_gemm_workspace_bytes", "mega_conv_gemm_clustered", "mega_set_tf32_rounding",
     "mega_conv_chain_plan_bytes", "mega_conv_chain_encode", "mega_conv_chain_launch", "mega_conv_chain_set_trace",
     "mega_conv_chain_encode2", "mega_conv_chain_launch2", "mega_set_split3_seg_len", "mega_conv_chain_set_trace2", "mega_nms_host", "mega_roi_align_forward_nchw_host",
     "mega_nms_workspace_bytes", "mega_nms", "mega_rpn_select_workspace_bytes", "mega_rpn_select",
diff --git a/mega.pytorch_b200/mega_core/b200/ops.py b/mega.pytorch_b200/mega_core/b200/ops.py
--- a/mega.pytorch_b200/mega_core/b200/ops.py
+++ b/mega.pytorch_b200/mega_core/b200/ops.py
@@ -40,9 +40,10 @@
 
 
 def _desc_info(d):
-    return {"m": d.n_img * d.out_h * d.out_w, "batch": d.batch, "cout": d.cout, "k": d.k_per_tap,
+    m_tiles = d.n_img * -(-d.out_h // d.tile_h) * -(-d.out_w // d.tile_w) if d.tile_h * d.tile_w else 0
+    return {"m": d.n_img * d.out_h * d.out_w, "m_tiles": m_tiles, "batch": d.batch, "cout": d.cout, "k": d.k_per_tap,
             "taps": d.taps_r * d.taps_s, "bn": d.block_n, "sk": d.stream_k, "res": bool(d.residual), "out16": d.out_f16,
-            "precision": d.precision}
+            "precision": d.precision, "cluster": bool(lib.mega_conv_gemm_clustered(ctypes.byref(d)))}
 
 
 _CHAIN_MODE = [None]
```
